# alexrich021/3dvnet

Hardware: AMD Instinct MI355X
Metric: depth maps/sec (256x320, 96 planes, 7 src) (higher is better)
Workload: dtype f32 storage/accumulate; MFMA operands split-bf16x3 (hi*hi+hi*lo+lo*hi, 16 mantissa bits); warp/variance f32 VALU; 1 GPU; cfg2: ScanNet-shape 256x320, 1 ref + 7 src (8 edges/ref), 96 planes, 56x56 plane grid, 32-ch quarter features 64x80; fused warp+variance -> CostRegNet -> soft-argmin depth (rows A1-A6); n_img_per_gpu=71, edges_per_ref=8, parallelism=single GPU, launch=eager, ranks_seen=1

## Files before the change

### 3dvnet_amd/_lib.py

```python
import ctypes
import os

import torch

_HERE = os.path.dirname(os.path.abspath(__file__))
LIB_PATH = os.path.join(_HERE, 'lib3dvnet_hip.so')
ABI_VERSION = 9
PRECISION = {'split_bf16': 0, 'fp32': 1}
LAYOUT = {'reference': 0, 'split': 1, 'cl8': 2}


def precision_code(name):
    try:
        return PRECISION[name]
    except KeyError:
        raise ValueError("precision must be 'split_bf16' or 'fp32', got %r" % (name,))


c_void_p, c_int, c_float, c_double, c_size_t = (ctypes.c_void_p, ctypes.c_int, ctypes.c_float,
                                                ctypes.c_double, ctypes.c_size_t)
c_float_p = ctypes.POINTER(ctypes.c_float)
c_float_pp = ctypes.POINTER(c_float_p)

SIGNATURES = {
    'v3d_version': (c_int, []),
    'v3d_last_error': (ctypes.c_char_p, []),
    'v3d_set_option': (c_int, [ctypes.c_char_p, c_int]),
    'v3d_get_option': (c_int, [ctypes.c_char_p, ctypes.POINTER(c_int)]),
    'v3d_timing_enable': (c_int, [c_int]),
    'v3d_timing_collect': (c_int, [c_int, ctypes.c_char_p, c_int, ctypes.POINTER(c_float),
                                   ctypes.POINTER(c_int)]),
    'v3d_psv_workspace_bytes': (c_size_t, [c_int] * 4),
    'v3d_psv_walk_chunks': (c_int, [c_int] * 4),
    'v3d_psv_variance_f32': (c_int, [c_void_p] * 7 + [c_int] * 8 + [c_double] * 2 + [c_int] * 3 +
                             [c_void_p, c_void_p, c_size_t, c_void_p]),
    'v3d_psv_sample_positions_f32': (c_int, [c_void_p] * 6 + [c_int] * 7 + [c_double] * 2 + [c_int] * 3 +
                                     [c_void_p, c_void_p, c_void_p, c_size_t, c_void_p]),
    'v3d_psv_variance_split': (c_int, [c_void_p] * 7 + [c_int] * 8 + [c_double] * 2 + [c_int] * 3 +
                               [c_void_p, c_void_p, c_size_t, c_void_p]),
    'v3d_psv_variance_cl8': (c_int, [c_void_p] * 7 + [c_int] * 8 + [c_double] * 2 + [c_int] * 3 +
                             [c_void_p, c_void_p, c_size_t, c_void_p]),
    'v3d_costreg_depth_cl8': (c_int, [c_void_p] * 3 + [c_int] * 4 + [c_void_p, c_void_p, c_void_p,
                                                                    c_size_t, c_void_p]),
    'v3d_costreg_pack': (c_int, [c_float_pp] * 5 + [c_float_p, c_float_p, c_int, c_int, c_float,
                                                     ctypes.POINTER(c_void_p)]),
    'v3d_costreg_free': (None, [c_void_p]),
    'v3d_costreg_workspace_bytes': (c_size_t, [c_void_p] + [c_int] * 4),
    'v3d_costreg_depth_f32': (c_int, [c_void_p] * 3 + [c_int] * 4 + [c_void_p, c_void_p, c_int, c_void_p,
                                                                    c_size_t, c_void_p]),
    'v3d_costreg_depth_split': (c_int, [c_void_p] * 3 + [c_int] * 4 + [c_void_p, c_void_p, c_void_p,
                                                                      c_size_t, c_void_p]),
    'v3d_costreg_layer_f32': (c_int, [c_void_p, c_int, c_void_p, c_void_p] + [c_int] * 4 +
                              [c_void_p, c_int, c_void_p]),
    'v3d_costreg_layer_split_workspace_bytes': (c_size_t, [c_int] * 5),
    'v3d_costreg_layer_split_f32': (c_int, [c_void_p, c_int, c_void_p, c_void_p] + [c_int] * 4 +
                                    [c_void_p, c_void_p, c_size_t, c_void_p]),
    'v3d_propagation_pack': (c_int, [c_float_pp] * 5 + [c_int, c_int, c_float, ctypes.POINTER(c_void_p)]),
    'v3d_propagation_free': (None, [c_void_p]),
    'v3d_propagation_up_f32': (c_int, [c_void_p, c_void_p, c_void_p] + [c_int] * 6 + [c_void_p, c_void_p, c_void_p, c_int, c_void_p]),
    'v3d_backproject_workspace_bytes': (c_size_t, [c_int] * 4),
    'v3d_backproject_variance_f32': (c_int, [c_void_p] * 8 + [c_int] * 10 + [c_double, c_int] +
                                     [c_void_p, c_void_p, c_void_p, c_size_t, c_void_p]),
    'v3d_gemm_pack': (c_int, [c_float_p, ctypes.c_longlong, ctypes.c_longlong, ctypes.c_longlong,
                              c_int, c_int, c_int, c_float_p, c_float_p, c_float_p, c_float_p,
                              ctypes.POINTER(c_void_p)]),
    'v3d_gemm_free': (None, [c_void_p]),
    'v3d_gemm_gather_f32': (c_int, [c_void_p, c_int, ctypes.POINTER(c_void_p), ctypes.POINTER(c_void_p),
                                    ctypes.POINTER(c_int), c_int, c_int, c_int, c_float, c_void_p, c_int,
                                    c_int, c_void_p, c_void_p, c_int, c_void_p, c_int, c_int, c_void_p]),
    'v3d_sparse_conv_f32': (c_int, [c_void_p, c_int, c_void_p, c_int, c_void_p, ctypes.c_longlong, c_int, c_float, c_void_p,
                                    c_int, c_int, c_void_p, c_int, c_int, c_void_p]),
    'v3d_fill_f32': (c_int, [c_void_p, c_size_t, c_float, c_void_p]),
    'v3d_pointnet_input_f32': (c_int, [c_void_p] * 5 + [c_int, c_int, c_void_p, c_void_p]),
    'v3d_hash_bytes': (c_size_t, [c_int]),
    'v3d_hash_build': (c_int, [c_void_p, c_int, c_void_p, c_size_t, c_void_p]),
    'v3d_hash_status': (c_int, [c_void_p, c_int, c_void_p]),
    'v3d_sparse_neighbors': (c_int, [c_void_p, c_int, c_void_p, c_int, c_int, c_void_p, c_void_p]),
    'v3d_sparse_interp_workspace_bytes': (c_size_t, [c_int, c_int]),
    'v3d_sparse_interp_f32': (c_int, [c_void_p, c_int, c_void_p, c_int, c_int, c_void_p, c_void_p, c_int,
                                      c_int, c_void_p, c_float, c_void_p, c_int, c_int, c_void_p, c_size_t,
                                      c_void_p]),
    'v3d_edges_csr_workspace_bytes': (c_size_t, [c_int, c_int]),
    'v3d_edges_csr': (c_int, [c_void_p, c_int, c_int, c_int, c_void_p, c_void_p, c_void_p, c_void_p, c_size_t, c_void_p]),
    'v3d_edges_csr_status': (c_int, [c_void_p, c_size_t, c_void_p]),
    'v3d_segment_csr_workspace_bytes': (c_size_t, [c_int]),
    'v3d_segment_csr': (c_int, [c_void_p, c_int, c_int, c_void_p, c_void_p, c_void_p, c_size_t, c_void_p]),
    'v3d_segment_max_f32': (c_int, [c_void_p, c_int, c_void_p, c_void_p, c_int, c_int, c_void_p, c_int, c_void_p]),
    'v3d_sort_unique_workspace_bytes': (c_size_t, [c_int]),
    'v3d_sort_unique_u64': (c_int, [c_void_p, c_int, c_void_p, ctypes.POINTER(c_int), c_void_p, c_size_t, c_void_p]),
    'v3d_strided_keys': (c_int, [c_void_p, c_int, c_int, c_void_p, c_void_p]),
    'v3d_unpack_coords': (c_int, [c_void_p, c_int, c_void_p, c_void_p]),
    'v3d_voxelize_workspace_bytes': (c_size_t, []),
    'v3d_voxel_keys': (c_int, [c_void_p, c_void_p, c_int, c_float, c_void_p, c_void_p, c_size_t, c_void_p]),
    'v3d_voxelize_status': (c_int, [c_void_p, c_size_t, c_void_p]),
    'v3d_lower_bound_u64': (c_int, [c_void_p, c_int, c_void_p, c_int, c_void_p, c_void_p]),
    'v3d_voxel_decode': (c_int, [c_void_p, c_int, c_float, c_float, c_void_p, c_void_p, c_void_p, c_void_p,
                                 c_size_t, c_void_p]),
    'v3d_decoder_fused_f32': (c_int, [ctypes.POINTER(c_void_p), c_void_p, c_void_p, ctypes.POINTER(c_void_p),
                                      ctypes.POINTER(c_int), ctypes.POINTER(c_void_p), ctypes.POINTER(c_int),
                                      ctypes.POINTER(c_int), ctypes.POINTER(c_void_p), ctypes.POINTER(c_float), c_void_p,
                                      c_void_p, c_void_p, c_int, c_int, c_int, c_void_p, c_void_p, c_void_p, c_void_p, c_void_p,
                                      c_size_t, c_void_p]),
    'v3d_decoder_fused_workspace_bytes': (c_size_t, [c_int, c_int]),
    'v3d_conv_pack': (c_int, [c_float_p, c_float_p, c_int, c_int, ctypes.POINTER(c_void_p)]),
    'v3d_conv_free': (None, [c_void_p]),
    'v3d_conv_nhwc_f32': (c_int, [c_void_p, c_void_p] + [c_int] * 7 + [c_void_p, c_void_p, c_void_p]),
    'v3d_depthwise_nhwc_f32': (c_int, [c_void_p] * 3 + [c_int] * 7 + [c_void_p, c_void_p]),
    'v3d_stem_f32': (c_int, [c_void_p] * 3 + [c_int] * 3 + [c_void_p, c_void_p]),
    'v3d_nhwc_to_nchw_f32': (c_int, [c_void_p, c_void_p, c_int, c_int, c_int, c_void_p]),
    'v3d_irb_pack': (c_int, [c_float_p] * 6 + [c_int] * 6 + [ctypes.POINTER(c_void_p)]),
    'v3d_irb_free': (None, [c_void_p]),
    'v3d_irb_supported': (c_int, [c_void_p, c_int, c_int]),
    'v3d_irb_workspace_bytes': (c_size_t, [c_void_p, c_int, c_int, c_int]),
    'v3d_stem_block_pack': (c_int, [c_float_p] * 6 + [ctypes.POINTER(c_void_p)]),
    'v3d_stem_block_f32': (c_int, [c_void_p, c_void_p, c_int, c_int, c_int, c_void_p, c_void_p]),
    'v3d_irb_nhwc_f32': (c_int, [c_void_p, c_void_p, c_int, c_int, c_int, c_void_p, c_void_p, c_size_t, c_void_p]),
    'v3d_fpn_pack': (c_int, [c_float_p] * 4 + [c_int, ctypes.POINTER(c_void_p)]),
    'v3d_fpn_free': (None, [c_void_p]),
    'v3d_fpn_level_f32': (c_int, [c_void_p, c_void_p, c_void_p, c_int, c_int, c_int, c_void_p, c_void_p, c_void_p]),
    'v3d_decoder_head_f32': (c_int, [c_void_p, c_int, c_int, c_int, c_void_p, c_void_p, c_void_p, c_void_p,
                                     c_void_p, c_void_p]),
    'v3d_fusion_workspace_bytes': (c_size_t, [c_int] * 3),
    'v3d_fuse_depths_f32': (c_int, [c_void_p, c_void_p, c_int, c_int, c_int, ctypes.POINTER(c_int), c_int, ctypes.POINTER(c_int),
                                    ctypes.POINTER(c_int), c_double, c_void_p, c_void_p, c_void_p, c_size_t, c_void_p]),
    'v3d_fusion_compact': (c_int, [c_void_p, c_void_p, c_void_p] + [c_int] * 5 + [c_void_p] * 7 + [c_size_t, c_void_p]),
    'v3d_cloud_downsample_workspace_bytes': (c_size_t, [c_int]),
    'v3d_cloud_downsample_f32': (c_int, [c_void_p, c_void_p, c_int, c_int, c_void_p, c_double, c_void_p, c_void_p, c_void_p,
                                         c_void_p, c_size_t, c_void_p]),
    'v3d_cloud_status': (c_int, [c_void_p, c_size_t, ctypes.POINTER(c_int), c_void_p]),
    'v3d_nn_workspace_bytes': (c_size_t, [c_int, c_int]),
    'v3d_nn_query_f32': (c_int, [c_void_p, c_int, c_void_p, c_int, c_void_p, c_void_p, c_void_p, c_size_t, c_void_p]),
    'v3d_cloud_metrics_workspace_bytes': (c_size_t, []),
    'v3d_cloud_metrics_f64': (c_int, [c_void_p, c_int, c_void_p, c_int, c_double, c_void_p, c_void_p, c_size_t, c_void_p]),
    'v3d_tsdf_integrate_f32': (c_int, [c_void_p, c_void_p, c_void_p, c_int, c_int, c_int, c_double, c_float_p, c_double, c_void_p,
                                       c_void_p, c_void_p, c_int, c_int, c_int, c_void_p]),
    'v3d_tsdf_normalize_f32': (c_int, [c_void_p, c_void_p, c_void_p, c_int, c_void_p, c_void_p, c_void_p]),
    'v3d_mesh_workspace_bytes': (c_size_t, [c_int, c_int, c_int]),
    'v3d_mesh_count_f32': (c_int, [c_void_p, c_int, c_int, c_int, c_int, c_void_p, c_void_p, c_size_t, c_void_p]),
    'v3d_mesh_extract_f32': (c_int, [c_void_p, c_void_p, c_int, c_int, c_int, c_double, c_float_p, c_int, c_void_p, c_void_p, c_int,
                                     c_void_p, c_int, c_void_p, c_size_t, c_void_p]),
    'v3d_mesh_render_depth_f32': (c_int, [c_void_p, c_int, c_void_p, c_int, c_void_p, c_int, c_int, c_int, c_double, c_double,
                                          c_double, c_void_p, c_void_p, c_void_p]),
    'v3d_tsdf_resample_f32': (c_int, [c_void_p, c_void_p, c_int, c_int, c_int, c_int, c_double, c_float_p, c_float_p, c_int, c_int,
                                      c_int, c_int, c_float_p, c_void_p, c_void_p, c_void_p]),
    'v3d_volume_resample_nearest': (c_int, [c_void_p, c_int, c_int, c_int, c_int, c_int, c_double, c_float_p, c_float_p, c_int, c_int,
                                            c_int, c_int, c_float_p, c_int, c_void_p, c_void_p, c_void_p]),
    'v3d_costreg_depth_prob': (c_int, [c_void_p, c_void_p, c_int, c_int, c_void_p, c_double, c_double] + [c_int] * 4 +
                               [c_void_p, c_void_p, c_void_p, c_void_p, c_size_t, c_void_p]),
    'v3d_soft_argmin_f32': (c_int, [c_void_p, c_void_p, c_double, c_double] + [c_int] * 4 + [c_void_p, c_void_p, c_void_p]),
    'v3d_confidence_logits_f32': (c_int, [c_void_p, c_void_p, c_double, c_double] + [c_int] * 4 + [c_void_p, c_void_p]),
    'v3d_probability_map_f32': (c_int, [c_void_p, c_void_p, c_double, c_double] + [c_int] * 4 + [c_void_p, c_void_p]),
    'v3d_depth_metrics_workspace_bytes': (c_size_t, [c_int] * 3),
    'v3d_depth_metrics_2d': (c_int, [c_void_p, c_int, c_int, c_void_p, c_void_p, c_void_p, c_int, c_void_p, c_int] + [c_int] * 3 +
                             [c_void_p, c_void_p, c_void_p, c_void_p, c_size_t, c_void_p]),
    'v3d_depth_supervision_workspace_bytes': (c_size_t, [c_int] * 3),
    'v3d_depth_supervision_f32': (c_int, [c_void_p, c_int, c_int, c_int, c_void_p, c_int, c_int, c_void_p, c_void_p, c_float] +
                                  [c_void_p, c_void_p, c_void_p, c_void_p, c_size_t, c_void_p]),
    'v3d_order_stats_workspace_bytes': (c_size_t, [c_int]),
    'v3d_backproject_order_stats_f32': (c_int, [c_void_p, c_void_p, c_int, c_int, c_int, ctypes.POINTER(c_double), c_int, c_void_p,
                                                c_void_p, c_void_p, c_size_t, c_void_p]),
    'v3d_cloud_order_stats_f32': (c_int, [c_void_p, c_int, ctypes.POINTER(c_double), c_int, c_void_p, c_void_p, c_void_p, c_size_t,
                                          c_void_p]),
}


class V3DLibraryError(RuntimeError):
    """lib3dvnet_hip.so is missing / unloadable, or a call returned an error code."""


_ERR_NAMES = {-1: 'V3D_ERR_BAD_SHAPE', -2: 'V3D_ERR_BAD_ARG', -3: 'V3D_ERR_WORKSPACE_TOO_SMALL',
              -4: 'V3D_ERR_HIP', -5: 'V3D_ERR_UNSUPPORTED'}
_lib = None


def load():
    global _lib
    if _lib is not None:
        return _lib
    if not os.path.exists(LIB_PATH):
        raise V3DLibraryError('%s not found: the HIP extension is not built (run '
                              '`python 3dvnet_amd/build.py`); there is no CPU fallback' % LIB_PATH)
    try:
        lib = ctypes.CDLL(LIB_PATH)
    except OSError as e:
        raise V3DLibraryError('cannot load %s: %s' % (LIB_PATH, e))
    for name, (res, args) in SIGNATURES.items():
        try:
            fn = getattr(lib, name)
        except AttributeError:
            raise V3DLibraryError('%s does not export %s' % (LIB_PATH, name))
        fn.restype = res
        fn.argtypes = args
    if lib.v3d_version() != ABI_VERSION:
        raise V3DLibraryError('ABI version mismatch: library %d, binding %d'
# ... 53 lines not shown
```

### 3dvnet_amd/csrc/costreg.hip

```cpp
#include <cstdlib>
#include <type_traits>
#include <vector>

#include "v3d_common.h"
#include "weight_pack.h"

#ifndef V3D_ABLATE
#define V3D_ABLATE 0
#endif

namespace {

typedef float f32x4 __attribute__((ext_vector_type(4)));
typedef float f32x2 __attribute__((ext_vector_type(2)));

enum { kConvS1 = 0, kConvS2 = 1, kDeconvS2 = 2, kConvS1Pair = 3 };

#ifdef V3D_PHASE_TIMING
constexpr int kPhaseSlots = 1 << 16;
__device__ unsigned long long g_phase[8 * kPhaseSlots];
#define PHASE_DECL                                  \
  long long ph_t = __builtin_readcyclecounter();    \
  long long ph_acc[8] = {0, 0, 0, 0, 0, 0, 0, 0}
#define PHASE_MARK(i)                                   \
// ... 1396 lines not shown
    for (int j = 0; j < 4; ++j) acc[i][j] = (f32x4){0.f, 0.f, 0.f, 0.f};
#pragma unroll
  for (int cbi = 0; cbi < NCBI; ++cbi) {
    const int cb = wave + 8 * cbi;
    if (cb < C9::NCB && V3D_C9_ABLATE != 3) {
      const int cz = cb / C9::CY, cy = cb % C9::CY;
#pragma unroll
      for (int dz = 0; dz < 2; ++dz)
#pragma unroll
        for (int dy = 0; dy < 2; ++dy) {
          if constexpr (F32) {
            float bv[8];
#pragma unroll
            for (int sl = 0; sl < 8; ++sl)
              bv[sl] = xf[(4 * (sl & 3) + kq) * C9::FS + ((cz + dz) * C9::VY + (cy + dy)) * C9::VX + jn + (sl >> 2)];
#pragma unroll
            for (int pz = 0; pz < 2; ++pz)
#pragma unroll
              for (int py = 0; py < 2; ++py) {
                if ((pz == 0 || dz == 1) && (py == 0 || dy == 1)) {
                  const int blk = (pz == 1 ? 2 : dz) * 3 + (py == 1 ? 2 : dy);
                  const f32x4 a0 = *reinterpret_cast<const f32x4*>(wff + ((blk * 2 + 0) * 64 + lane) * 4);
                  const f32x4 a1 = *reinterpret_cast<const f32x4*>(wff + ((blk * 2 + 1) * 64 + lane) * 4);
                  f32x4& c = acc[cbi][pz * 2 + py];
#pragma unroll
                  for (int sl = 0; sl < 8; ++sl)
                    c = __builtin_amdgcn_mfma_f32_16x16x4f32(sl < 4 ? a0[sl] : a1[sl - 4], bv[sl], c, 0, 0, 0);
                }
              }
            continue;
          }
          const int slot = (((cz + dz) * C9::VY + (cy + dy)) * C9::VX + jn + (kq >> 1)) * 2 + (kq & 1);
          const bf16x8 b_hi = __builtin_bit_cast(bf16x8, xh[slot]);
          const bf16x8 b_lo = __builtin_bit_cast(bf16x8, xl[slot]);
#pragma unroll
          for (int pz = 0; pz < 2; ++pz)
#pragma unroll
            for (int py = 0; py < 2; ++py) {
              if ((pz == 0 || dz == 1) && (py == 0 || dy == 1)) {
                const int blk = (pz == 1 ? 2 : dz) * 3 + (py == 1 ? 2 : dy);
                const bf16x8 a_hi = __builtin_bit_cast(bf16x8, wfr[(blk * 2) * 64 + lane]);
                const bf16x8 a_lo = __builtin_bit_cast(bf16x8, wfr[(blk * 2 + 1) * 64 + lane]);
                f32x4& c = acc[cbi][pz * 2 + py];
                c = __builtin_amdgcn_mfma_f32_16x16x32_bf16(a_hi, b_hi, c, 0, 0, 0);
                c = __builtin_amdgcn_mfma_f32_16x16x32_bf16(a_hi, b_lo, c, 0, 0, 0);
                c = __builtin_amdgcn_mfma_f32_16x16x32_bf16(a_lo, b_hi, c, 0, 0, 0);
              }
            }
        }
    }
  }
  PHASE_MARK(2);
  __syncthreads();
  PHASE_MARK(3);

  {
    float bias[4];
#pragma unroll
    for (int r = 0; r < 4; ++r) bias[r] = p.bias9[cbase + r];
#pragma unroll
    for (int cbi = 0; cbi < NCBI; ++cbi) {
      const int cb = wave + 8 * cbi;
      if (cb < C9::NCB && jn < C9::CX) {
        const int cz = cb / C9::CY, cy = cb % C9::CY;
#pragma unroll
        for (int rb = 0; rb < 4; ++rb) {
          const int hz = 2 * cz + (rb >> 1), hy = 2 * cy + (rb & 1), hx = 2 * jn + px;
          const int gz = oz0 - 1 + hz, gy = oy0 - 1 + hy, gx = ox0 - 1 + hx;
          const bool inside = gz >= 0 && gz < p.D && gy >= 0 && gy < p.H && gx >= 0 && gx < p.W;
          float skv[4];
          if constexpr (F32) {
#pragma unroll
            for (int r = 0; r < 4; ++r) skv[r] = skf[cbi][rb][r];
          } else {
            const u32x2 sh = skh[cbi][rb], sl = skl[cbi][rb];
            skv[0] = __uint_as_float(sh.x << 16) + __uint_as_float(sl.x << 16);
            skv[1] = __uint_as_float(sh.x & 0xffff0000u) + __uint_as_float(sl.x & 0xffff0000u);
            skv[2] = __uint_as_float(sh.y << 16) + __uint_as_float(sl.y << 16);
            skv[3] = __uint_as_float(sh.y & 0xffff0000u) + __uint_as_float(sl.y & 0xffff0000u);
          }
          float val[4];
#pragma unroll
          for (int r = 0; r < 4; ++r) val[r] = inside ? fmaxf(acc[cbi][rb][r] + bias[r], 0.f) + skv[r] : 0.f;
#pragma unroll
          for (int rp = 0; rp < 2; ++rp)
            *reinterpret_cast<f32x2*>(u9s + ((((cbase >> 1) + rp) * (C9::HD * C9::HH) + hz * C9::HH + hy) * C9::RS + hx) * 2) =
                (f32x2){val[2 * rp], val[2 * rp + 1]};
        }
      }
    }
  }
  PHASE_MARK(4);
  __syncthreads();
  PHASE_MARK(5);

  {
    const int z = wave >> 1, y = (wave & 1) * 4 + (lane >> 4), xp = lane & 15;
    if (xp < C9::TW / 2) {
      f32x2 o0[3] = {{0.f, 0.f}, {0.f, 0.f}, {0.f, 0.f}}, o1[3] = {{0.f, 0.f}, {0.f, 0.f}, {0.f, 0.f}};
      const f32x2* wp2 = reinterpret_cast<const f32x2*>(p.wprob);
#pragma unroll 1
      for (int cp = 0; cp < (V3D_C9_ABLATE == 1 ? 0 : V3D_C9_ABLATE == 2 ? 1 : 4); ++cp) {
#pragma unroll
        for (int ky = 0; ky < 3; ++ky) {
#pragma unroll
          for (int kz = 0; kz < 3; ++kz) {
            const f32x2* row = reinterpret_cast<const f32x2*>(u9s) +
                               (cp * (C9::HD * C9::HH) + (z + kz) * C9::HH + (y + ky)) * C9::RS + 2 * xp;
            const f32x4 q0 = *reinterpret_cast<const f32x4*>(row), q1 = *reinterpret_cast<const f32x4*>(row + 2);
            const f32x2 a0 = {q0.x, q0.y}, a1 = {q0.z, q0.w}, a2 = {q1.x, q1.y}, a3 = {q1.z, q1.w};
            const f32x2* wk = wp2 + (cp * 27 + (kz * 3 + ky) * 3);
            const f32x2 w0 = wk[0], w1 = wk[1], w2 = wk[2];
            o0[kz] += a0 * w0; o1[kz] += a1 * w0;
            o0[kz] += a1 * w1; o1[kz] += a2 * w1;
            o0[kz] += a2 * w2; o1[kz] += a3 * w2;
          }
        }
      }
      const f32x2 s0 = (o0[0] + o0[1]) + o0[2], s1 = (o1[0] + o1[1]) + o1[2];
      const int gz = oz0 + z, gy = oy0 + y, gx = ox0 + 2 * xp;
      if (gz < p.D && gy < p.H && gx < p.W) {
        const float bsv = p.bprob[0];
        const f32x2 res = {s0.x + s0.y + bsv, s1.x + s1.y + bsv};
        float* o = p.out + ((size_t)n * out_plane + (size_t)(gz * p.H) * p.W) + (unsigned)(__umul24(gy, p.W) + gx);
        if (gx + 1 < p.W && (p.W & 1) == 0) {
          *reinterpret_cast<f32x2*>(o) = res;
        } else {
          o[0] = res.x;
          if (gx + 1 < p.W) o[1] = res.y;
        }
      }
    }
  }
  PHASE_MARK(6);
  PHASE_FLUSH;
}

__global__ __launch_bounds__(256) void encode_split_kernel(const float* __restrict__ in, u32x4* __restrict__ out, int C,
                                                           size_t plane, size_t total) {
  const size_t i = (size_t)blockIdx.x * 256 + threadIdx.x;
  if (i >= total) return;
  const size_t sp = i % plane, ng = i / plane;
  const float* src = in + (ng * 8) * plane + sp;
  float v[8];
#pragma unroll
  for (int c = 0; c < 8; ++c) v[c] = src[(size_t)c * plane];
  u32x2 ha, la, hb, lb;
  split4(v[0], v[1], v[2], v[3], ha, la);
  split4(v[4], v[5], v[6], v[7], hb, lb);
  out[(ng * 2) * plane + sp] = (u32x4){ha.x, ha.y, hb.x, hb.y};
  out[(ng * 2 + 1) * plane + sp] = (u32x4){la.x, la.y, lb.x, lb.y};
}

__global__ __launch_bounds__(256) void soft_argmin_kernel(const float* __restrict__ reg,
                                                          const float* __restrict__ vals,
                                                          float* __restrict__ depth, int n, int D,
                                                          int HW) {
  const size_t gid = (size_t)blockIdx.x * 256 + threadIdx.x;
  if (gid >= (size_t)n * HW) return;
  const int b = gid / HW, pix = gid % HW;
  const float* col = reg + (size_t)b * D * HW + pix;
  float m = -INFINITY, num = 0.f, den = 0.f;
  auto step = [&](float xin, float val) __attribute__((always_inline)) {
    const float x = -xin;
    if (x > m) {
      const float sc = expf(m - x);
      num *= sc; den *= sc; m = x;
    }
    const float ex = expf(x - m);
    num += val * ex;
    den += ex;
  };
  int d = 0;
  for (; d + 8 <= D; d += 8) {
    float x[8];
#pragma unroll
    for (int i = 0; i < 8; ++i) x[i] = __builtin_nontemporal_load(col + (size_t)(d + i) * HW);
#pragma unroll
    for (int i = 0; i < 8; ++i) step(x[i], vals[d + i]);
  }
  for (; d < D; ++d) step(col[(size_t)d * HW], vals[d]);
  const float e = num / den;
  depth[gid] = e;
}

#ifndef V3D_L0_CFG
#define V3D_L0_CFG kConvS1Pair, 32, 8, 4, 8, 28, 4, 3
#endif
typedef ConvCfg<V3D_L0_CFG> L0;
typedef ConvCfg<kConvS1Pair, 16, 8, 4, 8, 28, 4, 3> L0_16;
#ifndef V3D_L1_CFG
#define V3D_L1_CFG kConvS2, 8, 16, 2, 4, 28, 4
#endif
typedef ConvCfg<V3D_L1_CFG> L1;
#ifndef V3D_L2_CFG
#define V3D_L2_CFG kConvS1, 16, 16, 4, 4, 28, 8
#endif
typedef ConvCfg<V3D_L2_CFG> L2;
typedef ConvCfg<kConvS2, 16, 32, 2, 7, 14, 4> L3;
typedef ConvCfg<kConvS1, 32, 32, 4, 7, 14, 8> L4;
typedef ConvCfg<kConvS2, 32, 64, 2, 4, 7, 8> L5;
typedef ConvCfg<kConvS1, 64, 64, 2, 4, 7, 16> L6;
typedef ConvCfg<kDeconvS2, 64, 32, 4, 8, 14, 16> L7;
#ifndef V3D_L8_CFG
#define V3D_L8_CFG kDeconvS2, 32, 16, 4, 8, 28, 8
#endif
typedef ConvCfg<V3D_L8_CFG> L8;
#ifndef V3D_L9_CFG
#define V3D_L9_CFG kDeconvS2, 16, 8, 4, 8, 28, 16, 3
#endif
typedef ConvCfg<V3D_L9_CFG> L9;

struct LayerDesc { int mode, cin, cout, ck; };
const LayerDesc kLayers[10] = {
    {L0::MODE, 32, 8, L0::CK},   {L1::MODE, 8, 16, L1::CK},   {L2::MODE, 16, 16, L2::CK},
    {kConvS2, 16, 32, L3::CK},  {kConvS1, 32, 32, L4::CK},  {kConvS2, 32, 64, L5::CK},
    {kConvS1, 64, 64, L6::CK},  {kDeconvS2, 64, 32, L7::CK}, {kDeconvS2, 32, 16, L8::CK},
    {kDeconvS2, 16, 8, L9::CK}};

template <class C>
int launch_conv(const char* name, const float* in, const float* wp, const float* bias,
                const float* skip, float* out, int n, int Di, int Hi, int Wi, hipStream_t s) {
  ConvParams p;
  p.in = in; p.wp = wp; p.bias = bias; p.skip = skip; p.out = out; p.n = n;
  p.Di = Di; p.Hi = Hi; p.Wi = Wi;
  if (C::S1LIKE) { p.Do = Di; p.Ho = Hi; p.Wo = Wi; }
  else if (C::MODE == kConvS2) { p.Do = (Di - 1) / 2 + 1; p.Ho = (Hi - 1) / 2 + 1; p.Wo = (Wi - 1) / 2 + 1; }
  else { p.Do = 2 * Di; p.Ho = 2 * Hi; p.Wo = 2 * Wi; }
  p.ntz = (p.Do + C::TD - 1) / C::TD; p.nty = (p.Ho + C::TH - 1) / C::TH; p.ntx = (p.Wo + C::TW - 1) / C::TW;
  p.relu = 1;
  p.zy_order = 0;
  const long long blocks = (long long)n * p.ntz * p.nty * p.ntx;
  V3D_REQUIRE(blocks > 0 && blocks < (1ll << 31), V3D_ERR_BAD_SHAPE, "conv3d: bad grid");
  V3D_REQUIRE((long long)C::CK * Di * Hi * Wi < (1ll << 31), V3D_ERR_BAD_SHAPE,
              "conv3d: input volume too large for 32-bit tile offsets");
  {
    v3d::TimedScope ts(name, s);
    constexpr bool kVecOk = C::MODE == kConvS1Pair && C::PF && C::TW % 4 == 0 && C::IW <= 61;
    const bool vec = kVecOk && Wi % 4 == 0 && (reinterpret_cast<size_t>(in) & 15) == 0;
    if constexpr (kVecOk) {
      if (vec) conv3d_mfma_kernel<C, true><<<(unsigned)blocks, 256, 0, s>>>(p);
      else conv3d_mfma_kernel<C, false><<<(unsigned)blocks, 256, 0, s>>>(p);
    } else {
      conv3d_mfma_kernel<C, false><<<(unsigned)blocks, 256, 0, s>>>(p);
    }
  }
  V3D_CHECK_LAUNCH("conv3d_mfma_kernel");
  return V3D_OK;
}

}

namespace {
#ifndef V3D_C0_WAVES
#define V3D_C0_WAVES 8
#endif
constexpr int kC0Waves = V3D_C0_WAVES;
int launch_conv0_bf16(bool split_in, bool split_out, const float* in, const float* wbf, const float* bias, const float* skip, float* out, int n,
                      int Di, int Hi, int Wi, hipStream_t s) {
  ConvParams p;
  p.in = in; p.wp = wbf; p.bias = bias; p.skip = skip; p.out = out; p.n = n;
  p.Di = Di; p.Hi = Hi; p.Wi = Wi; p.Do = Di; p.Ho = Hi; p.Wo = Wi;
  p.ntz = (Di + C0::TD - 1) / C0::TD; p.nty = (Hi + C0::TH - 1) / C0::TH; p.ntx = (Wi + C0::TW - 1) / C0::TW;
  p.relu = 1;
  p.zy_order = tile_order(p.ntx, p.nty);
  const long long blocks = (long long)n * p.ntz * p.nty * p.ntx;
  V3D_REQUIRE(blocks > 0 && blocks < (1ll << 31), V3D_ERR_BAD_SHAPE, "conv0: bad grid");
  V3D_REQUIRE((long long)8 * Di * Hi * Wi < (1ll << 31), V3D_ERR_BAD_SHAPE, "conv0: input volume too large");
  static bool lds_opted[4][64] = {};
  const void* const kernels[4] = {(const void*)conv0_bf16x2_kernel<false, false, 4>, (const void*)conv0_bf16x2_kernel<true, false, 4>,
                                  (const void*)conv0_bf16x2_kernel<true, true, kC0Waves>, (const void*)conv0_bf16x2_kernel<false, true, 4>};
  for (int k = 0; k < 4; ++k)
    if (const int rc = v3d::opt_in_dynamic_lds(kernels[k], (int)C0::LDS_BYTES, lds_opted[k]); rc != V3D_OK) return rc;
  {
    v3d::TimedScope ts("costreg_conv0", s);
#ifdef V3D_C0_PERSIST
    const unsigned grid = v3d::persistent_grid(blocks, 2);
#else
    const unsigned grid = (unsigned)((blocks + 7) / 8 * 8);
#endif
    if (split_in && split_out) conv0_bf16x2_kernel<true, true, kC0Waves><<<grid, 64 * kC0Waves, C0::LDS_BYTES, s>>>(p);
    else if (split_in) conv0_bf16x2_kernel<true, false, 4><<<grid, 256, C0::LDS_BYTES, s>>>(p);
    else if (split_out) conv0_bf16x2_kernel<false, true, 4><<<grid, 256, C0::LDS_BYTES, s>>>(p);
    else conv0_bf16x2_kernel<false, false, 4><<<grid, 256, C0::LDS_BYTES, s>>>(p);
  }
  V3D_CHECK_LAUNCH("conv0_bf16x2_kernel");
  return V3D_OK;
}
}

namespace {
template <class C>
int launch_convg(const char* name, const void* in, const float* wbf, const float* bias, float* out_f32, void* out_split,
                 int n, int Di, int Hi, int Wi, hipStream_t s) {
  ConvGParams p;
  p.in = in; p.wp = wbf; p.bias = bias; p.out_f32 = out_f32; p.out_split = out_split; p.n = n;
  p.Di = Di; p.Hi = Hi; p.Wi = Wi;
  p.Do = (Di - 1) / C::S + 1; p.Ho = (Hi - 1) / C::S + 1; p.Wo = (Wi - 1) / C::S + 1;
  p.ntz = (p.Do + C::TD - 1) / C::TD; p.nty = (p.Ho + C::TH - 1) / C::TH; p.ntx = (p.Wo + C::TW - 1) / C::TW;
  const long long blocks = (long long)n * p.ntz * p.nty * p.ntx;
  V3D_REQUIRE(blocks > 0 && blocks < (1ll << 31), V3D_ERR_BAD_SHAPE, "%s: bad grid", name);
  V3D_REQUIRE(((C::OUT & kOutF32) == 0 || out_f32) && ((C::OUT & kOutSplit) == 0 || out_split), V3D_ERR_BAD_ARG,
              "%s: missing output buffer", name);
  p.m_tx = v3d::magic_u32((unsigned long long)blocks, (unsigned)p.ntx);
  p.m_ty = v3d::magic_u32((unsigned long long)blocks / p.ntx + 1, (unsigned)p.nty);
  p.m_tz = v3d::magic_u32((unsigned long long)blocks / p.ntx / p.nty + 1, (unsigned)p.ntz);
  V3D_REQUIRE(Di < (1 << 12) && Hi < (1 << 12) && Wi < (1 << 12) && (long long)Di * Hi * Wi < (1ll << 24), V3D_ERR_BAD_SHAPE,
              "%s: volume %d x %d x %d too large for 32-bit slot offsets", name, Di, Hi, Wi);
  static bool lds_opted[64] = {};
  if (const int rc = v3d::opt_in_dynamic_lds((const void*)convg_bf16x2_kernel<C>, (int)C::LDS_BYTES, lds_opted); rc != V3D_OK) return rc;
  {
    v3d::TimedScope ts(name, s);
    unsigned grid = (unsigned)((blocks * C::NCG + 7) / 8 * 8);
    if (C::PERSIST) {
      static int wgs_per_cu = 0;
      if (wgs_per_cu == 0) {
        int nb = 0;
        V3D_CHECK_HIP(hipOccupancyMaxActiveBlocksPerMultiprocessor(&nb, (const void*)convg_bf16x2_kernel<C>, 256, C::LDS_BYTES));
        wgs_per_cu = nb > 0 ? nb : 1;
      }
      grid = v3d::persistent_grid(blocks * C::NCG, wgs_per_cu);
    }
    convg_bf16x2_kernel<C><<<grid, 256, C::LDS_BYTES, s>>>(p, p.bias);
  }
  V3D_CHECK_LAUNCH(name);
  return V3D_OK;
}
}

namespace {
template <class C>
int launch_deconvg(const char* name, const void* in, const float* wbf, const float* bias, const float* skip, float* out_f32,
                   void* out_split, int n, int Di, int Hi, int Wi, hipStream_t s) {
  DeconvGParams p;
// ... 134 lines not shown

void pack_prob(const float* prob_w, float* out) {
  for (int cp = 0; cp < 4; ++cp)
    for (int t = 0; t < 27; ++t)
      for (int e = 0; e < 2; ++e) out[((size_t)cp * 27 + t) * 2 + e] = prob_w[(cp * 2 + e) * 27 + t];
}
}

extern "C" int v3d_costreg_pack(const float* const* conv_w, const float* const* bn_w,
                                const float* const* bn_b, const float* const* bn_m,
                                const float* const* bn_v, const float* prob_w, const float* prob_b,
                                int in_channels, int base, float eps,
                                v3d_costreg_weights** out_handle) {
  V3D_REQUIRE(conv_w && bn_w && bn_b && bn_m && bn_v && prob_w && prob_b && out_handle,
              V3D_ERR_BAD_ARG, "v3d_costreg_pack: null argument");
  V3D_REQUIRE((in_channels == 32 || in_channels == 16) && base == 8, V3D_ERR_UNSUPPORTED,
              "v3d_costreg_pack: CostRegNet(32, 8) and CostRegNet(16, 8) are built (got %d, %d)", in_channels, base);
  v3d_costreg_weights* h = new v3d_costreg_weights();
  h->in_channels = in_channels; h->base = base;
  v3d::HostImage img;
  std::vector<float> wf[10];
  for (int l = 0; l < 10; ++l) {
    LayerDesc L = kLayers[l];
    if (l == 0) L.cin = in_channels;
    const v3d::BnFold bn(bn_w[l], bn_b[l], bn_m[l], bn_v[l], eps, L.cout);
    wf[l] = L.mode == kDeconvS2 ? bn.weights(conv_w[l], L.cin, 27) : bn.weights(conv_w[l], 1, (size_t)L.cin * 27);
    h->wp_ofs[l] = img.reserve(tile_image_floats(L));
    h->bias_ofs[l] = img.reserve(L.cout);
    pack_tile_image(L, wf[l].data(), img.at(h->wp_ofs[l]));
    memcpy(img.at(h->bias_ofs[l]), bn.bias.data(), L.cout * sizeof(float));
  }
  h->c0bf_ofs = img.reserve((size_t)C0::NCH * C0::WU32);
  pack_conv0_split(wf[0].data(), in_channels, img.words(h->c0bf_ofs));
  h->c0f32_ofs = img.reserve((size_t)4 * 9 * 8 * 64);
  pack_conv0_f32(wf[0].data(), in_channels, img.at(h->c0f32_ofs));
  h->c9bf_ofs = img.reserve((size_t)C9::WU32);
  h->c9f32_ofs = img.reserve((size_t)C9::WF32);
  pack_conv9(wf[9].data(), img.words(h->c9bf_ofs), img.at(h->c9f32_ofs));
  for (int l = 1; l <= 8; ++l) {
    const int cin = kLayers[l].cin, cout = kLayers[l].cout;
    size_t& ofs = l <= 6 ? h->cgbf_ofs[l] : h->dgbf_ofs[l - 7];
    ofs = img.reserve((size_t)(cout / 16) * (cin / 8) * (l <= 6 ? 9 : 12) * 2 * kLoWords);
    if (l <= 6) pack_convg(wf[l].data(), cin, cout, img.words(ofs));
    else pack_deconvg(wf[l].data(), cin, cout, img.words(ofs));
  }
  h->prob_w2_ofs = img.reserve((size_t)base * 27);
  pack_prob(prob_w, img.at(h->prob_w2_ofs));
  h->prob_b_ofs = img.reserve(1);
  *img.at(h->prob_b_ofs) = prob_b[0];
  h->total = img.data.size();
  return v3d::finish_pack(h, img.data.data(), h->total * sizeof(float), "weights", out_handle);
}

extern "C" void v3d_costreg_free(v3d_costreg_weights* h) { v3d::release(h); }

static int run_layer(const v3d_costreg_weights* h, int layer, const float* in, const float* skip,
                     float* out, int n, int Di, int Hi, int Wi, int precision, hipStream_t s) {
  const float* wp = h->dev + h->wp_ofs[layer];
  const float* bias = h->dev + h->bias_ofs[layer];
  switch (layer) {
    case 0: {
      if (h->in_channels == 16) {
        V3D_REQUIRE(precision == V3D_PRECISION_FP32, V3D_ERR_UNSUPPORTED,
                    "costreg: the per-layer conv0 of CostRegNet(16, 8) is built for V3D_PRECISION_FP32 only (the chain entry points "
                    "cover both precisions)");
        return launch_conv<L0_16>("costreg_conv0", in, wp, bias, skip, out, n, Di, Hi, Wi, s);
      }
      if (precision == V3D_PRECISION_FP32) return launch_conv<L0>("costreg_conv0", in, wp, bias, skip, out, n, Di, Hi, Wi, s);
      return launch_conv0_bf16(false, false, in, h->dev + h->c0bf_ofs, bias, skip, out, n, Di, Hi, Wi, s);
    }
    case 1: return launch_conv<L1>("costreg_conv1", in, wp, bias, skip, out, n, Di, Hi, Wi, s);
    case 2: return launch_conv<L2>("costreg_conv2", in, wp, bias, skip, out, n, Di, Hi, Wi, s);
    case 3: return launch_conv<L3>("costreg_conv3", in, wp, bias, skip, out, n, Di, Hi, Wi, s);
    case 4: return launch_conv<L4>("costreg_conv4", in, wp, bias, skip, out, n, Di, Hi, Wi, s);
    case 5: return launch_conv<L5>("costreg_conv5", in, wp, bias, skip, out, n, Di, Hi, Wi, s);
    case 6: return launch_conv<L6>("costreg_conv6", in, wp, bias, skip, out, n, Di, Hi, Wi, s);
    case 7: return launch_conv<L7>("costreg_conv7", in, wp, bias, skip, out, n, Di, Hi, Wi, s);
    case 8: return launch_conv<L8>("costreg_conv8", in, wp, bias, skip, out, n, Di, Hi, Wi, s);
    case 9: return launch_conv<L9>("costreg_conv9", in, wp, bias, skip, out, n, Di, Hi, Wi, s);
  }
  return v3d::fail(V3D_ERR_BAD_ARG, "costreg: layer %d out of range", layer);
}

extern "C" int v3d_costreg_layer_f32(const v3d_costreg_weights* h, int layer, const float* in,
                                     const float* skip, int n, int Di, int Hi, int Wi, float* out,
                                     int precision, void* stream) {
  V3D_REQUIRE(h && in && out, V3D_ERR_BAD_ARG, "v3d_costreg_layer_f32: null argument");
  V3D_REQUIRE(n > 0 && Di > 0 && Hi > 0 && Wi > 0, V3D_ERR_BAD_SHAPE, "v3d_costreg_layer_f32: bad shape");
  V3D_REQUIRE(precision == V3D_PRECISION_SPLIT_BF16 || precision == V3D_PRECISION_FP32, V3D_ERR_BAD_ARG,
              "v3d_costreg_layer_f32: unknown precision %d", precision);
  return run_layer(h, layer, in, skip, out, n, Di, Hi, Wi, precision, (hipStream_t)stream);
}

extern "C" size_t v3d_costreg_layer_split_workspace_bytes(int n, int cin, int Di, int Hi, int Wi) {
  if (n <= 0 || cin <= 0 || Di <= 0 || Hi <= 0 || Wi <= 0) return 0;
  return v3d::align_up((size_t)n * cin * Di * Hi * Wi * sizeof(float), 256);
}

extern "C" int v3d_costreg_layer_split_f32(const v3d_costreg_weights* h, int layer, const float* in, const float* skip,
                                           int n, int Di, int Hi, int Wi, float* out, void* workspace,
                                           size_t workspace_bytes, void* stream) {
  static const int cins[9] = {32, 8, 16, 16, 32, 32, 64, 64, 32};
  V3D_REQUIRE(h && in && out && workspace, V3D_ERR_BAD_ARG, "v3d_costreg_layer_split_f32: null argument");
  V3D_REQUIRE(layer >= 1 && layer <= 8, V3D_ERR_BAD_ARG, "v3d_costreg_layer_split_f32: layer %d (1..8: conv1..conv8)", layer);
  V3D_REQUIRE(n > 0 && Di > 0 && Hi > 0 && Wi > 0, V3D_ERR_BAD_SHAPE, "v3d_costreg_layer_split_f32: bad shape");
  V3D_REQUIRE(layer < 7 || skip, V3D_ERR_BAD_ARG, "v3d_costreg_layer_split_f32: conv7 / conv8 need the skip tensor");
  const int cin = cins[layer];
  V3D_REQUIRE(workspace_bytes >= v3d_costreg_layer_split_workspace_bytes(n, cin, Di, Hi, Wi), V3D_ERR_WORKSPACE_TOO_SMALL,
              "v3d_costreg_layer_split_f32: workspace too small");
  hipStream_t s = (hipStream_t)stream;
  const size_t plane = (size_t)Di * Hi * Wi, total = (size_t)n * (cin / 8) * plane;
  encode_split_kernel<<<(unsigned)((total + 255) / 256), 256, 0, s>>>(in, (u32x4*)workspace, cin, plane, total);
  V3D_CHECK_LAUNCH("encode_split_kernel");
  const float* w = h->dev + (layer <= 6 ? h->cgbf_ofs[layer] : h->dgbf_ofs[layer - 7]);
  const float* bias = h->dev + h->bias_ofs[layer];
  switch (layer) {
    case 1: return launch_convg<CG<8, 16, 2, 14, kOutF32>>("costreg_conv1", workspace, w, bias, out, nullptr, n, Di, Hi, Wi, s);
    case 2: return launch_convg<CG<16, 16, 1, 14, kOutF32>>("costreg_conv2", workspace, w, bias, out, nullptr, n, Di, Hi, Wi, s);
    case 3: return launch_convg<CG<16, 32, 2, 14, kOutF32>>("costreg_conv3", workspace, w, bias, out, nullptr, n, Di, Hi, Wi, s);
    case 4: return launch_convg<CG<32, 32, 1, 14, kOutF32>>("costreg_conv4", workspace, w, bias, out, nullptr, n, Di, Hi, Wi, s);
    case 5: return launch_convg<CG<32, 64, 2, 8, kOutF32>>("costreg_conv5", workspace, w, bias, out, nullptr, n, Di, Hi, Wi, s);
    case 6: return launch_convg<CG<64, 64, 1, 8, kOutF32>>("costreg_conv6", workspace, w, bias, out, nullptr, n, Di, Hi, Wi, s);
    case 7: return launch_deconvg<DG<64, 32, 8, kOutF32>>("costreg_conv7", workspace, w, bias, skip, out, nullptr, n, Di, Hi, Wi, s);
    default: return launch_deconvg<DG<32, 16, 14, kOutF32>>("costreg_conv8", workspace, w, bias, skip, out, nullptr, n, Di, Hi, Wi, s);
  }
}

namespace {
struct WsPlan { size_t c0, c1, c2, c3, c4, c5, c6, u7, u8, u9, reg, enc, total; };
WsPlan plan_ws(int n, int D, int h, int w) {
  const size_t V0 = (size_t)D * h * w, V1 = V0 / 8, V2 = V1 / 8, V3 = V2 / 8;
  WsPlan p; size_t o = 0;
  auto take = [&](size_t nf) { size_t r = o; o += v3d::align_up(nf * sizeof(float), 256); return r; };
  p.c0 = take(n * 8 * V0); p.c1 = take(n * 16 * V1); p.c2 = take(n * 16 * V1);
  p.c3 = take(n * 32 * V2); p.c4 = take(n * 32 * V2); p.c5 = take(n * 64 * V3);
  p.c6 = take(n * 64 * V3); p.u7 = take(n * 32 * V2); p.u8 = take(n * 16 * V1);
  p.u9 = take(n * 8 * V0); p.reg = take(n * V0);
  p.enc = take(32 * V0);
  p.total = o;
  return p;
}
}

extern "C" size_t v3d_costreg_workspace_bytes(const v3d_costreg_weights*, int n_ref, int D, int h, int w) {
  if (n_ref <= 0 || D <= 0 || h <= 0 || w <= 0) return 0;
  return plan_ws(n_ref, D, h, w).total;
}

namespace {
int launch_soft_argmin(const float* xreg, const float* depth_vals, float* depth, int n, int D, int H, int W, hipStream_t s) {
  const size_t npix = (size_t)n * H * W;
  {
    v3d::TimedScope ts("soft_argmin", s);
    soft_argmin_kernel<<<(unsigned)((npix + 255) / 256), 256, 0, s>>>(xreg, depth_vals, depth, n, D, H * W);
  }
  V3D_CHECK_LAUNCH("soft_argmin_kernel");
  return V3D_OK;
}

struct ProbOut {
  float* prob = nullptr;
  double depth_start = 0., depth_interval = 0.;
};

int launch_depth_tail(const float* xreg, const float* depth_vals, float* depth, const ProbOut& po, int n, int D, int H, int W,
                      hipStream_t s) {
  if (!po.prob) return launch_soft_argmin(xreg, depth_vals, depth, n, D, H, W, s);
  return v3d::launch_soft_argmin_prob(xreg, depth_vals, depth, po.prob, po.depth_start, po.depth_interval, n, D, H, W, s);
}

int launch_conv9_prob(bool f32, const v3d_costreg_weights* h, const float* u8, const float* c0, float* xreg, int n, int D, int H, int W,
                      hipStream_t s) {
  C9Params q;
  q.u8 = u8; q.c0 = c0; q.wbf = h->dev + (f32 ? h->c9f32_ofs : h->c9bf_ofs); q.bias9 = h->dev + h->bias_ofs[9];
  q.wprob = h->dev + h->prob_w2_ofs; q.bprob = h->dev + h->prob_b_ofs; q.out = xreg;
  q.n = n; q.D = D; q.H = H; q.W = W;
  q.ntz = (D + C9::TD - 1) / C9::TD; q.nty = (H + C9::TH - 1) / C9::TH; q.ntx = (W + C9::TW - 1) / C9::TW;
  q.zy_order = tile_order(q.ntx, q.nty);
  const long long blocks = (long long)n * q.ntz * q.nty * q.ntx;
  V3D_REQUIRE(blocks < (1ll << 31), V3D_ERR_BAD_SHAPE, "conv9+prob: grid too large");
  V3D_REQUIRE((long long)D * H * W < (1ll << 26) && D < (1 << 12) && H < (1 << 12) && W < (1 << 12), V3D_ERR_BAD_SHAPE,
              "conv9+prob: volume %d x %d x %d too large for 32-bit offsets", D, H, W);
  q.m_tx = v3d::magic_u32((unsigned long long)blocks, (unsigned)q.ntx);
  q.m_t1 = v3d::magic_u32((unsigned long long)blocks / q.ntx + 1, (unsigned)(q.zy_order ? q.ntz : q.nty));
  q.m_t2 = v3d::magic_u32((unsigned long long)blocks / q.ntx / (q.zy_order ? q.ntz : q.nty) + 1, (unsigned)(q.zy_order ? q.nty : q.ntz));
  {
    v3d::TimedScope ts(f32 ? "costreg_conv9_prob_f32" : "costreg_conv9_prob", s);
    if (f32) conv9_prob_kernel<true><<<(unsigned)blocks, 512, 0, s>>>(q);
    else conv9_prob_kernel<false><<<(unsigned)blocks, 512, 0, s>>>(q);
  }
  V3D_CHECK_LAUNCH("conv9_prob_kernel");
  return V3D_OK;
}

int run_split_tail(const v3d_costreg_weights* h, const WsPlan& ws, char* base, const float* depth_vals, int n, int D, int H, int W,
                   float* depth, float* xreg, const ProbOut& po, hipStream_t s) {
  const size_t V1 = (size_t)D * H * W / 8;
  auto F = [&](size_t o) { return (float*)(base + o); };
  float* const c2s = F(ws.u9);
  float* const c4s = c2s + (size_t)n * 16 * V1;
  auto W_ = [&](int l) { return h->dev + h->cgbf_ofs[l]; };
  auto B_ = [&](int l) { return h->dev + h->bias_ofs[l]; };
#ifdef V3D_PHASE_TIMING
  const int stop_after = v3d::option(v3d::kOptStopAfter);
#else
  const int stop_after = 99;
#endif
  int rc = V3D_OK;
  if (stop_after < 1) return rc;
  if (v3d::option(v3d::kOptC12March) != 0) {
    rc = v3d::launch_conv12z(F(ws.c0), W_(1), W_(2), B_(1), B_(2), c2s, n, D, H, W, s);
  } else if ((rc = launch_convg<CG<8, 16, 2, 14, kOutSplit>>("costreg_conv1", F(ws.c0), W_(1), B_(1), nullptr, F(ws.c1), n, D, H, W,
                                                              s)) == V3D_OK) {
    rc = launch_convg<CG<16, 16, 1, 14, kOutSplit>>("costreg_conv2", F(ws.c1), W_(2), B_(2), nullptr, c2s, n, D / 2, H / 2, W / 2, s);
  }
  if (rc != V3D_OK || stop_after < 3) return rc;
  if ((rc = launch_convg<CG<16, 32, 2, 14, kOutSplit>>("costreg_conv3", c2s, W_(3), B_(3), nullptr, F(ws.c3), n, D / 2, H / 2, W / 2,
                                                       s)) != V3D_OK || stop_after < 4) return rc;
  if ((rc = launch_convg<CG<32, 32, 1, 14, kOutSplit>>("costreg_conv4", F(ws.c3), W_(4), B_(4), nullptr, c4s, n, D / 4, H / 4, W / 4,
                                                       s)) != V3D_OK || stop_after < 5) return rc;
  if ((rc = launch_convg<CG<32, 64, 2, 8, kOutSplit>>("costreg_conv5", c4s, W_(5), B_(5), nullptr, F(ws.c5), n, D / 4, H / 4, W / 4,
                                                      s)) != V3D_OK || stop_after < 6) return rc;
  if ((rc = launch_convg<CG<64, 64, 1, 8, kOutSplit>>("costreg_conv6", F(ws.c5), W_(6), B_(6), nullptr, F(ws.c6), n, D / 8, H / 8,
                                                      W / 8, s)) != V3D_OK || stop_after < 7) return rc;
  if ((rc = launch_deconvg<DG<64, 32, 8, kOutSplit, true>>("costreg_conv7", F(ws.c6), h->dev + h->dgbf_ofs[0], B_(7), c4s, nullptr,
                                                           F(ws.u7), n, D / 8, H / 8, W / 8, s)) != V3D_OK || stop_after < 8) return rc;
  if ((rc = launch_deconvg<DG<32, 16, 14, kOutSplit, true>>("costreg_conv8", F(ws.u7), h->dev + h->dgbf_ofs[1], B_(8), c2s, nullptr,
                                                            F(ws.u8), n, D / 4, H / 4, W / 4, s)) != V3D_OK || stop_after < 9) return rc;
  if ((rc = launch_conv9_prob(false, h, F(ws.u8), F(ws.c0), xreg, n, D, H, W, s)) != V3D_OK || stop_after < 10) return rc;
  return launch_depth_tail(xreg, depth_vals, depth, po, n, D, H, W, s);
}
}

static int costreg_depth_impl(int in_layout, const v3d_costreg_weights* h, const float* var,
                              const float* depth_vals, int n, int D, int H, int W,
                              float* depth, float* reg, int precision, void* workspace,
                              size_t workspace_bytes, void* stream, const ProbOut& po = ProbOut()) {
  V3D_REQUIRE(precision == V3D_PRECISION_SPLIT_BF16 || precision == V3D_PRECISION_FP32, V3D_ERR_BAD_ARG,
              "v3d_costreg_depth_f32: unknown precision %d", precision);
  V3D_REQUIRE(h && var && depth_vals && depth && workspace, V3D_ERR_BAD_ARG,
              "v3d_costreg_depth_f32: null argument");
  V3D_REQUIRE(n > 0 && D > 0 && H > 0 && W > 0 && D % 8 == 0 && H % 8 == 0 && W % 8 == 0,
              V3D_ERR_BAD_SHAPE, "v3d_costreg_depth_f32: D,h,w must be positive multiples of 8 (got %d,%d,%d)", D, H, W);
  const WsPlan ws = plan_ws(n, D, H, W);
  V3D_REQUIRE(workspace_bytes >= ws.total, V3D_ERR_WORKSPACE_TOO_SMALL,
              "v3d_costreg_depth_f32: workspace %zu < %zu", workspace_bytes, ws.total);
  hipStream_t s = (hipStream_t)stream;
  char* base = (char*)workspace;
  auto F = [&](size_t o) { return (float*)(base + o); };
  float* xreg = reg ? reg : F(ws.reg);
  int rc;
#define RUN(layer, in, skip, out, d, hh, ww) \
  if ((rc = run_layer(h, layer, in, skip, out, n, d, hh, ww, V3D_PRECISION_FP32, s)) != V3D_OK) return rc;
  const bool generic = precision == V3D_PRECISION_FP32;
  const bool split_in = in_layout == 1, cl8_in = in_layout == 2;
  V3D_REQUIRE(!generic || !split_in, V3D_ERR_UNSUPPORTED, "V3D_PRECISION_FP32 needs an fp32 variance volume");
  V3D_REQUIRE(h->in_channels == 32 || in_layout == 0, V3D_ERR_UNSUPPORTED,
              "CostRegNet(16, 8) takes the variance volume in the reference layout (the hand-off formats are defined for 32 channels)");
  V3D_REQUIRE(generic || !cl8_in, V3D_ERR_UNSUPPORTED, "the fp32 channel-last volume is the input of V3D_PRECISION_FP32");
  if (generic) {
    if (cl8_in) {
      if ((rc = v3d::launch_conv0z(true, var, h->dev + h->c0f32_ofs, h->dev + h->bias_ofs[0], F(ws.c0), n, D, H, W, s)) != V3D_OK)
        return rc;
    } else {
      RUN(0, var, nullptr, F(ws.c0), D, H, W);
    }
    RUN(1, F(ws.c0), nullptr, F(ws.c1), D, H, W);
    RUN(2, F(ws.c1), nullptr, F(ws.c2), D / 2, H / 2, W / 2);
  } else {
    if (split_in) {
      if ((rc = v3d::launch_conv0z(false, var, h->dev + h->c0bf_ofs, h->dev + h->bias_ofs[0], F(ws.c0), n, D, H, W, s)) != V3D_OK) return rc;
    } else {
      const int cin = h->in_channels, ngrp = cin / 8;
      const size_t V0 = (size_t)D * H * W, total = (size_t)ngrp * V0;
      if (ngrp < 4) V3D_CHECK_HIP(hipMemsetAsync((char*)F(ws.enc) + (size_t)ngrp * 2 * V0 * 16, 0, (size_t)(4 - ngrp) * 2 * V0 * 16, s));
      for (int i = 0; i < n; ++i) {
        encode_split_kernel<<<(unsigned)((total + 255) / 256), 256, 0, s>>>(var + (size_t)i * cin * V0, (u32x4*)F(ws.enc), cin, V0, total);
        V3D_CHECK_LAUNCH("encode_split_kernel");
        if ((rc = v3d::launch_conv0z(false, F(ws.enc), h->dev + h->c0bf_ofs, h->dev + h->bias_ofs[0], F(ws.c0) + (size_t)i * 8 * V0, 1, D, H,
                                     W, s)) != V3D_OK) return rc;
      }
    }
    return run_split_tail(h, ws, base, depth_vals, n, D, H, W, depth, xreg, po, s);
  }
  RUN(3, F(ws.c2), nullptr, F(ws.c3), D / 2, H / 2, W / 2);
  RUN(4, F(ws.c3), nullptr, F(ws.c4), D / 4, H / 4, W / 4);
  RUN(5, F(ws.c4), nullptr, F(ws.c5), D / 4, H / 4, W / 4);
  RUN(6, F(ws.c5), nullptr, F(ws.c6), D / 8, H / 8, W / 8);
  RUN(7, F(ws.c6), F(ws.c4), F(ws.u7), D / 8, H / 8, W / 8);
  RUN(8, F(ws.u7), F(ws.c2), F(ws.u8), D / 4, H / 4, W / 4);
  if ((rc = launch_conv9_prob(true, h, F(ws.u8), F(ws.c0), xreg, n, D, H, W, s)) != V3D_OK) return rc;
#undef RUN
  return launch_depth_tail(xreg, depth_vals, depth, po, n, D, H, W, s);
}

extern "C" int v3d_costreg_depth_f32(const v3d_costreg_weights* h, const float* var, const float* depth_vals, int n,
                                     int D, int H, int W, float* depth, float* reg, int precision, void* workspace,
                                     size_t workspace_bytes, void* stream) {
  return costreg_depth_impl(0, h, var, depth_vals, n, D, H, W, depth, reg, precision, workspace, workspace_bytes,
                            stream);
}

extern "C" int v3d_costreg_depth_cl8(const v3d_costreg_weights* h, const void* var_cl8, const float* depth_vals,
                                     int n, int D, int H, int W, float* depth, float* reg, void* workspace,
                                     size_t workspace_bytes, void* stream) {
  return costreg_depth_impl(2, h, (const float*)var_cl8, depth_vals, n, D, H, W, depth, reg, V3D_PRECISION_FP32, workspace,
                            workspace_bytes, stream);
}

extern "C" int v3d_costreg_depth_split(const v3d_costreg_weights* h, const void* var_split, const float* depth_vals,
                                       int n, int D, int H, int W, float* depth, float* reg, void* workspace,
                                       size_t workspace_bytes, void* stream) {
  return costreg_depth_impl(1, h, (const float*)var_split, depth_vals, n, D, H, W, depth, reg,
                            V3D_PRECISION_SPLIT_BF16, workspace, workspace_bytes, stream);
}

extern "C" int v3d_costreg_depth_prob(const v3d_costreg_weights* h, const void* var, int in_layout, int precision,
                                      const float* depth_vals, double depth_start, double depth_interval, int n, int D, int H,
                                      int W, float* depth, float* reg, float* prob, void* workspace, size_t workspace_bytes,
                                      void* stream) {
  V3D_REQUIRE(in_layout == V3D_LAYOUT_REFERENCE || in_layout == V3D_LAYOUT_SPLIT || in_layout == V3D_LAYOUT_CL8, V3D_ERR_BAD_ARG,
              "v3d_costreg_depth_prob: unknown input layout %d", in_layout);
  const float ds = (float)depth_start, di = (float)depth_interval;
  V3D_REQUIRE(std::isfinite(ds) && std::isfinite(di) && di != 0.f, V3D_ERR_BAD_ARG,
              "v3d_costreg_depth_prob: depth_start = %g / depth_interval = %g must be finite fp32 numbers, the interval not zero",
              depth_start, depth_interval);
  V3D_REQUIRE(D < (1 << 24), V3D_ERR_BAD_SHAPE, "v3d_costreg_depth_prob: D = %d too large", D);
  ProbOut po;
  po.prob = prob; po.depth_start = depth_start; po.depth_interval = depth_interval;
  return costreg_depth_impl(in_layout, h, (const float*)var, depth_vals, n, D, H, W, depth, reg, precision, workspace,
                            workspace_bytes, stream, po);
}

extern "C" int v3d_soft_argmin_f32(const float* x_reg, const float* depth_vals, double depth_start, double depth_interval, int n,
                                   int D, int H, int W, float* depth, float* prob, void* stream) {
  V3D_REQUIRE(x_reg && depth_vals && depth, V3D_ERR_BAD_ARG, "v3d_soft_argmin_f32: null argument");
  V3D_REQUIRE(n > 0 && D > 0 && H > 0 && W > 0 && D < (1 << 24) && (long long)H * W < (1ll << 31) &&
                  ((long long)n * H * W + 255) / 256 < (1ll << 31),
              V3D_ERR_BAD_SHAPE, "v3d_soft_argmin_f32: n, D, h, w = %d, %d, %d, %d", n, D, H, W);
  const float ds = (float)depth_start, di = (float)depth_interval;
  V3D_REQUIRE(!prob || (std::isfinite(ds) && std::isfinite(di) && di != 0.f), V3D_ERR_BAD_ARG,
              "v3d_soft_argmin_f32: depth_start = %g / depth_interval = %g must be finite fp32 numbers, the interval not zero",
              depth_start, depth_interval);
  ProbOut po;
  po.prob = prob; po.depth_start = depth_start; po.depth_interval = depth_interval;
  return launch_depth_tail(x_reg, depth_vals, depth, po, n, D, H, W, (hipStream_t)stream);
}

#ifdef V3D_PHASE_TIMING
extern "C" int v3d_debug_phase_read(unsigned long long* out8_host, int n_blocks) {
  V3D_CHECK_HIP(hipDeviceSynchronize());
  std::vector<unsigned long long> h((size_t)8 * kPhaseSlots);
  V3D_CHECK_HIP(hipMemcpyFromSymbol(h.data(), HIP_SYMBOL(g_phase), h.size() * sizeof(unsigned long long)));
  for (int i = 0; i < 8; ++i) out8_host[i] = 0;
  for (int b = 0; b < n_blocks && b < kPhaseSlots; ++b)
    for (int i = 0; i < 8; ++i) out8_host[i] += h[(size_t)b * 8 + i];
  return V3D_OK;
}
#endif
```

### 3dvnet_amd/csrc/edges.hip

```cpp
#include "v3d_common.h"

namespace {

constexpr int kThreads = 1024, kWaves = kThreads / 64;

struct CsrMeta {
  int magic;
  int error;
  int n_ref;
  int pad;
};
constexpr int kMagic = 0x43535231;
constexpr int kLdsImgs = 4096, kLdsEdges = 8192;

__device__ __forceinline__ int block_inclusive_sum(int v, int* s_wave, int& total) {
  const int lane = threadIdx.x & 63, wave = threadIdx.x >> 6;
#pragma unroll
  for (int o = 1; o < 64; o <<= 1) {
    const int u = __shfl_up(v, o, 64);
    if (lane >= o) v += u;
  }
  __syncthreads();
  if (lane == 63) s_wave[wave] = v;
  __syncthreads();
  int base = 0, tot = 0;
#pragma unroll
  for (int w = 0; w < kWaves; ++w) {
    const int x = s_wave[w];
    if (w < wave) base += x;
    tot += x;
  }
  total = tot;
  return v + base;
}

__global__ __launch_bounds__(kThreads) void edges_csr_kernel(const long long* __restrict__ edges, int n_edges, int n_img,
                                                              int n_ref_expected, int* __restrict__ ref_img,
                                                              int* __restrict__ edge_ofs, int* __restrict__ edge_src,
                                                              CsrMeta* __restrict__ meta, int* rank,
                                                              int* __restrict__ count) {
  __shared__ int s_wave[kWaves];
  __shared__ int s_err;
  __shared__ int s_rank[kLdsImgs];
  __shared__ int s_er[kLdsEdges];
  const bool small = n_img <= kLdsImgs && n_edges <= kLdsEdges;
  if (small) rank = s_rank;
  const int tid = threadIdx.x, lane = tid & 63, wave = tid >> 6;
  const long long* const e_ref = edges;
  const long long* const e_src = edges + n_edges;
  if (tid == 0) s_err = 0;
  for (int i = tid; i < n_img; i += kThreads) rank[i] = 0;
  __syncthreads();
  int bad = 0;
  for (int e = tid; e < n_edges; e += kThreads) {
    const long long r = e_ref[e], s = e_src[e];
    if (r < 0 || r >= n_img || s < 0 || s >= n_img) bad = 1;
    else rank[r] = 1;
  }
  if (bad) s_err = 2;
  __syncthreads();
  const int per = (n_img + kThreads - 1) / kThreads;
  const int lo = min(tid * per, n_img), hi = min(lo + per, n_img);
  int sum = 0;
  for (int i = lo; i < hi; ++i) sum += rank[i];
  int n_ref;
  int run = block_inclusive_sum(sum, s_wave, n_ref) - sum;
  for (int i = lo; i < hi; ++i) {
    const int f = rank[i];
    rank[i] = f ? run : -1;
    if (f && run < n_ref_expected) ref_img[run] = i;
    run += f;
  }
  int err = s_err | (n_ref != n_ref_expected ? 1 : 0);
  if (tid == 0) { meta->magic = kMagic; meta->error = err; meta->n_ref = n_ref; }
  __syncthreads();
  if (err) {
    for (int r = tid; r <= n_ref_expected; r += kThreads) edge_ofs[r] = 0;
    for (int r = tid; r < n_ref_expected; r += kThreads) ref_img[r] = 0;
    return;
  }
  if (small) {
    for (int e = tid; e < n_edges; e += kThreads) s_er[e] = rank[e_ref[e]];
    __syncthreads();
  }
  auto edge_rank = [&](int e) __attribute__((always_inline)) { return small ? s_er[e] : rank[e_ref[e]]; };
  for (int r = wave; r < n_ref; r += kWaves) {
    int c = 0;
    for (int e0 = 0; e0 < n_edges; e0 += 64) {
      const int e = e0 + lane;
      const bool hit = e < n_edges && edge_rank(e) == r;
      c += __builtin_popcountll(__ballot(hit));
    }
    if (lane == 0) count[r] = c;
  }
  __syncthreads();
  const int per_r = (n_ref + kThreads - 1) / kThreads;
  const int rlo = min(tid * per_r, n_ref), rhi = min(rlo + per_r, n_ref);
  sum = 0;
  for (int r = rlo; r < rhi; ++r) sum += count[r];
  int n_counted;
  run = block_inclusive_sum(sum, s_wave, n_counted) - sum;
  for (int r = rlo; r < rhi; ++r) { edge_ofs[r] = run; run += count[r]; }
  if (tid == 0) edge_ofs[n_ref] = n_counted;
  __syncthreads();
  for (int r = wave; r < n_ref; r += kWaves) {
    int pos = edge_ofs[r];
    for (int e0 = 0; e0 < n_edges; e0 += 64) {
      const int e = e0 + lane;
      const bool hit = e < n_edges && edge_rank(e) == r;
      const unsigned long long m = __ballot(hit);
      if (hit) edge_src[pos + __builtin_popcountll(m & ((1ull << lane) - 1ull))] = (int)e_src[e];
      pos += __builtin_popcountll(m);
    }
  }
}

}

extern "C" size_t v3d_edges_csr_workspace_bytes(int n_img, int n_ref) {
  return sizeof(CsrMeta) + ((size_t)(n_img > 0 ? n_img : 0) + (size_t)(n_ref > 0 ? n_ref : 0)) * sizeof(int);
}

extern "C" int v3d_edges_csr(const int64_t* edges, int n_edges, int n_img, int n_ref, int32_t* ref_img, int32_t* edge_ofs,
                             int32_t* edge_src, void* workspace, size_t workspace_bytes, void* stream) {
  V3D_REQUIRE(edges && ref_img && edge_ofs && edge_src && workspace, V3D_ERR_BAD_ARG, "v3d_edges_csr: null pointer");
  V3D_REQUIRE(n_edges > 0 && n_img > 0 && n_ref > 0 && n_ref <= n_img, V3D_ERR_BAD_SHAPE,
              "v3d_edges_csr: n_edges=%d n_img=%d n_ref=%d", n_edges, n_img, n_ref);
  V3D_REQUIRE(workspace_bytes >= v3d_edges_csr_workspace_bytes(n_img, n_ref), V3D_ERR_WORKSPACE_TOO_SMALL,
              "v3d_edges_csr: workspace %zu < %zu bytes", workspace_bytes, v3d_edges_csr_workspace_bytes(n_img, n_ref));
  hipStream_t s = (hipStream_t)stream;
  CsrMeta* meta = (CsrMeta*)workspace;
  int* rank = (int*)(meta + 1);
  int* count = rank + n_img;
  {
    v3d::TimedScope ts("edges_csr", s);
    edges_csr_kernel<<<1, kThreads, 0, s>>>((const long long*)edges, n_edges, n_img, n_ref, ref_img, edge_ofs, edge_src, meta,
                                            rank, count);
  }
  V3D_CHECK_LAUNCH("edges_csr_kernel");
  return V3D_OK;
}

extern "C" int v3d_edges_csr_status(const void* workspace, size_t workspace_bytes, void* stream) {
  V3D_REQUIRE(workspace && workspace_bytes >= sizeof(CsrMeta), V3D_ERR_BAD_ARG, "v3d_edges_csr_status: not a CSR workspace");
  CsrMeta h;
  V3D_CHECK_HIP(hipMemcpyAsync(&h, workspace, sizeof(h), hipMemcpyDeviceToHost, (hipStream_t)stream));
  V3D_CHECK_HIP(hipStreamSynchronize((hipStream_t)stream));
  V3D_REQUIRE(h.magic == kMagic, V3D_ERR_BAD_ARG, "v3d_edges_csr_status: not a CSR workspace");
  V3D_REQUIRE((h.error & 2) == 0, V3D_ERR_BAD_SHAPE, "v3d_edges_csr: an edge names an image outside [0, n_img)");
  V3D_REQUIRE((h.error & 1) == 0, V3D_ERR_BAD_SHAPE,
              "v3d_edges_csr: the edge list holds %d distinct reference images, not the number the caller passed", h.n_ref);
  return V3D_OK;
}
```

### 3dvnet_amd/csrc/psv_variance.hip

```cpp
#include <cstdlib>

#include <vector>

#include "bf16_split.h"
#include "v3d_common.h"

namespace {

constexpr int kThreads = 256;
constexpr int kPix = 64;
constexpr int kDB = 4;
constexpr int kMaxE = 8;

struct PsvParams {
  const float* featT;
  const float* K;
  const float* R;
  const float* t;
  const int* ref_img;
  const int* edge_ofs;
  const int* edge_src;
  float* var;
  const float* camp;
  int n_img, n_ref, Hf, Wf, H, W, D, h, w, n_ptile;
  double x_step, y_step, z_start, z_step, z_end;
  float rWm1, rHm1;
  unsigned m_dseg, m_ptile, m_w;
  int n_dchunk, walk, n_dseg;
  int skip;
};


template <int C>
__global__ __launch_bounds__(256) void transpose_channel_last_kernel(const float* __restrict__ in,
                                                                      float* __restrict__ out,
                                                                      int HW) {
  __shared__ float tile[C][kPix + 1];
  const int img = blockIdx.y;
  const int p0 = blockIdx.x * kPix;
  const float* src = in + (size_t)img * C * HW;
  float* dst = out + (size_t)img * HW * C;
  for (int i = threadIdx.x; i < C * kPix; i += 256) {
    int c = i / kPix, p = i % kPix;
    tile[c][p] = (p0 + p < HW) ? src[(size_t)c * HW + p0 + p] : 0.f;
  }
  __syncthreads();
  for (int i = threadIdx.x; i < C * kPix; i += 256) {
    int p = i / C, c = i % C;
    if (p0 + p < HW) dst[(size_t)(p0 + p) * C + c] = tile[c][p];
  }
}

__host__ __device__ constexpr int kTailCells(int Wf) { return 2 * (Wf + 2) + 16; }

template <int C>
__global__ __launch_bounds__(256) void transpose_bordered_kernel(const float* __restrict__ in, float* __restrict__ out, int Hf,
                                                                  int Wf, int n_img) {
  __shared__ float tile[C][kPix + 1];
  const int img = blockIdx.y;
  const int Wp = Wf + 2, HW = Hf * Wf, n_cell = (Hf + 2) * Wp;
  const int q0 = blockIdx.x * kPix;
  const float* src = in + (size_t)img * C * HW;
  float* dst = out + (size_t)img * n_cell * C;
  for (int i = threadIdx.x; i < C * kPix; i += 256) {
    const int c = i / kPix, q = q0 + i % kPix;
    const int yb = q / Wp, xb = q - yb * Wp;
    const bool inside = q < n_cell && yb >= 1 && yb <= Hf && xb >= 1 && xb <= Wf;
    tile[c][i % kPix] = inside ? src[(size_t)c * HW + (yb - 1) * Wf + xb - 1] : 0.f;
  }
  __syncthreads();
  for (int i = threadIdx.x; i < C * kPix; i += 256) {
    const int px = i / C, c = i % C;
    if (q0 + px < n_cell) dst[(size_t)(q0 + px) * C + c] = tile[c][px];
  }
  if (img == n_img - 1 && blockIdx.x == 0) {
    float* tail = out + (size_t)n_img * n_cell * C;
    for (int i = threadIdx.x; i < kTailCells(Wf) * C; i += 256) tail[i] = 0.f;
  }
}

#ifdef V3D_PHASE_TIMING
constexpr int kPhaseSlots = 1 << 16;
__device__ unsigned long long g_psv_phase[8 * kPhaseSlots];
#define PHASE_DECL                                  \
  long long ph_t = __builtin_readcyclecounter();    \
  long long ph_acc[8] = {0, 0, 0, 0, 0, 0, 0, 0}
#define PHASE_MARK(i)                                   \
  do {                                                  \
    long long t_ = __builtin_readcyclecounter();        \
    ph_acc[i] += t_ - ph_t;                             \
    ph_t = t_;                                          \
  } while (0)
#define PHASE_FLUSH                                                                                       \
  do {                                                                                                    \
    if (threadIdx.x == 0 && blockIdx.x < kPhaseSlots)                                                     \
      for (int i_ = 0; i_ < 8; ++i_) g_psv_phase[blockIdx.x * 8 + i_] = (unsigned long long)ph_acc[i_];   \
  } while (0)
#else
#define PHASE_DECL
#define PHASE_MARK(i)
#define PHASE_FLUSH
#endif

constexpr int kCamStride = 36;

__global__ void cam_setup_kernel(const float* __restrict__ K, const float* __restrict__ R,
                                 const float* __restrict__ t, float* __restrict__ camp, int n_img) {
  const int img = blockIdx.x * blockDim.x + threadIdx.x;
  if (img >= n_img) return;
  const float* Kp = K + img * 9;
  const float* Rp = R + img * 9;
  const float* tp = t + img * 3;
  float* o = camp + img * kCamStride;
  double a = Kp[0], bb = Kp[1], c = Kp[2], d = Kp[3], e = Kp[4], f = Kp[5], g = Kp[6], hh = Kp[7], i = Kp[8];
  double det = a * (e * i - f * hh) - bb * (d * i - f * g) + c * (d * hh - e * g);
  double id = 1.0 / det;
  o[0] = (float)((e * i - f * hh) * id);
  o[1] = (float)((c * hh - bb * i) * id);
  o[2] = (float)((bb * f - c * e) * id);
  o[3] = (float)((f * g - d * i) * id);
  o[4] = (float)((a * i - c * g) * id);
  o[5] = (float)((c * d - a * f) * id);
  o[6] = (float)((d * hh - e * g) * id);
  o[7] = (float)((bb * g - a * hh) * id);
  o[8] = (float)((a * e - bb * d) * id);
  for (int k = 0; k < 9; ++k) o[9 + k] = Rp[k];
  for (int k = 0; k < 3; ++k) o[18 + k] = tp[k];
  for (int r = 0; r < 3; ++r)
    for (int j = 0; j < 4; ++j) {
      const float b0 = j < 3 ? Rp[0 * 3 + j] : tp[0], b1 = j < 3 ? Rp[1 * 3 + j] : tp[1], b2 = j < 3 ? Rp[2 * 3 + j] : tp[2];
      o[24 + r * 4 + j] = v3d::add_rn(v3d::add_rn(v3d::mul_rn(Kp[r * 3 + 0], b0), v3d::mul_rn(Kp[r * 3 + 1], b1)),
                                    v3d::mul_rn(Kp[r * 3 + 2], b2));
    }
}

struct TapInfo {
  float w00, w01, w10, w11;
  unsigned b00;
  unsigned pad[3];
};

template <unsigned CB>
__device__ __forceinline__ TapInfo make_taps(float ix, float iy, int Wf, int Hf, int first_cell) {
  ix = fminf(fmaxf(ix, -1.f), (float)Wf);
  iy = fminf(fmaxf(iy, -1.f), (float)Hf);
  const float x0 = floorf(ix), y0 = floorf(iy);
  const float x1 = x0 + 1.f, y1 = y0 + 1.f;
  const float wx0 = x1 - ix, wx1 = ix - x0, wy0 = y1 - iy, wy1 = iy - y0;
  TapInfo ti;
  ti.w00 = v3d::mul_rn(wx0, wy0); ti.w01 = v3d::mul_rn(wx1, wy0);
  ti.w10 = v3d::mul_rn(wx0, wy1); ti.w11 = v3d::mul_rn(wx1, wy1);
  ti.b00 = (unsigned)(first_cell + ((int)y0 + 1) * (Wf + 2) + (int)x0 + 1) * CB;
  return ti;
}

typedef float f32x4 __attribute__((ext_vector_type(4)));
typedef unsigned int u32x2 __attribute__((ext_vector_type(2)));
typedef unsigned int u32x4 __attribute__((ext_vector_type(4)));

using v3d::bf16_rne;
using v3d::pack_bf16x2;

template <int C, bool SPLIT>
__global__ __launch_bounds__(64) void psv_variance_kernel(PsvParams p) {
  constexpr int kThreads = 64, kPix = kThreads / 4;
  constexpr int LP = C / 4;
  constexpr int PPP = kThreads / LP;
  constexpr int NPASS = kPix / PPP;
  static_assert(kPix % PPP == 0, "tile");

  __shared__ TapInfo s_tap[kMaxE * kPix];
  __shared__ __attribute__((aligned(16))) float s_out[C][kPix + 1];
  __shared__ float s_ref[24];
  __shared__ float s_P[kMaxE][12];

  const int tid = threadIdx.x;
  const int n_dchunk = (p.D + kDB - 1) / kDB;
  int b = v3d::xcd_contiguous_block();
  const int ptile = b % p.n_ptile; b /= p.n_ptile;
  const int dchunk = b % n_dchunk;
  const int r = b / n_dchunk;
  const int P = p.h * p.w;
  const int e_begin = p.edge_ofs[r], e_end = p.edge_ofs[r + 1];
  const int ne = e_end - e_begin;
  const int ref = p.ref_img[r];

  if (tid < 21) s_ref[tid] = p.camp[ref * kCamStride + tid];

  const int cg = tid % LP;
  const int pix_in_pass = tid / LP;

  const int px1 = tid % kPix;
  const int gp1 = ptile * kPix + px1;
  float xf = 0.f, yf = 0.f;
  {
    int gy = gp1 / p.w, gx = gp1 % p.w;
    xf = (p.w > 1 && gx == p.w - 1) ? (float)(p.W - 1) : (float)((double)gx * p.x_step);
    yf = (p.h > 1 && gy == p.h - 1) ? (float)(p.H - 1) : (float)((double)gy * p.y_step);
  }
  const float Wm1 = (float)(p.W - 1), Hm1 = (float)(p.H - 1);
  const float rWm1 = (float)(1.0 / (double)(p.W - 1)), rHm1 = (float)(1.0 / (double)(p.H - 1));
  const float Wfm1 = (float)(p.Wf - 1), Hfm1 = (float)(p.Hf - 1);

  PHASE_DECL;
  for (int dd = 0; dd < kDB; ++dd) {
    const int d = dchunk * kDB + dd;
    if (d >= p.D) break;
    const float z = (d == p.D - 1 && p.D > 1) ? (float)p.z_end
                                               : (float)(p.z_start + (double)d * p.z_step);
    float acc_s[NPASS][4], acc_q[NPASS][4];
#pragma unroll
    for (int a = 0; a < NPASS; ++a)
#pragma unroll
      for (int k = 0; k < 4; ++k) acc_s[a][k] = acc_q[a][k] = 0.f;

    for (int ec = 0; ec < ne; ec += kMaxE) {
      const int nec = min(kMaxE, ne - ec);
      __syncthreads();
      PHASE_MARK(0);
      if (dd == 0 || ne > kMaxE) {
        for (int i = tid; i < nec * 12; i += kThreads)
          s_P[i / 12][i % 12] = p.camp[p.edge_src[e_begin + ec + i / 12] * kCamStride + 24 + i % 12];
      }
      __syncthreads();
      PHASE_MARK(1);
      {
        float X, Y, Z;
        v3d::world_point(s_ref, xf, yf, z, X, Y, Z);
        for (int e = tid / kPix; e < nec; e += kThreads / kPix) {
          float ix, iy;
          v3d::sample_position(s_P[e], X, Y, Z, Wm1, rWm1, Hm1, rHm1, Wfm1, Hfm1, ix, iy);
          const TapInfo ti = make_taps<4 * C>(ix, iy, p.Wf, p.Hf, p.edge_src[e_begin + ec + e] * (p.Hf + 2) * (p.Wf + 2));
          s_tap[e * kPix + px1] = ti;
        }
      }
      PHASE_MARK(2);
      __syncthreads();
      PHASE_MARK(3);
#pragma unroll
      for (int a = 0; a < NPASS; ++a) {
        const int px = a * PPP + pix_in_pass;
        for (int e = 0; e < nec; ++e) {
          const TapInfo ti = s_tap[e * kPix + px];
          float4 s;
          {
            const char* fb = reinterpret_cast<const char*>(p.featT);
            const unsigned cgb = cg * 16, rowb = (unsigned)(p.Wf + 2) * (4 * C);
            const float4 v00 = *reinterpret_cast<const float4*>(fb + (size_t)(ti.b00 + cgb));
            const float4 v01 = *reinterpret_cast<const float4*>(fb + (size_t)(ti.b00 + cgb) + 4 * C);
            const float4 v10 = *reinterpret_cast<const float4*>(fb + (size_t)(ti.b00 + rowb + cgb));
            const float4 v11 = *reinterpret_cast<const float4*>(fb + (size_t)(ti.b00 + rowb + cgb) + 4 * C);
            s.x = v3d::mul_rn(v00.x, ti.w00); s.y = v3d::mul_rn(v00.y, ti.w00);
            s.z = v3d::mul_rn(v00.z, ti.w00); s.w = v3d::mul_rn(v00.w, ti.w00);
            s.x = __builtin_fmaf(v01.x, ti.w01, s.x); s.y = __builtin_fmaf(v01.y, ti.w01, s.y);
            s.z = __builtin_fmaf(v01.z, ti.w01, s.z); s.w = __builtin_fmaf(v01.w, ti.w01, s.w);
            s.x = __builtin_fmaf(v10.x, ti.w10, s.x); s.y = __builtin_fmaf(v10.y, ti.w10, s.y);
            s.z = __builtin_fmaf(v10.z, ti.w10, s.z); s.w = __builtin_fmaf(v10.w, ti.w10, s.w);
            s.x = __builtin_fmaf(v11.x, ti.w11, s.x); s.y = __builtin_fmaf(v11.y, ti.w11, s.y);
            s.z = __builtin_fmaf(v11.z, ti.w11, s.z); s.w = __builtin_fmaf(v11.w, ti.w11, s.w);
          }
          acc_s[a][0] = v3d::add_rn(acc_s[a][0], s.x); acc_s[a][1] = v3d::add_rn(acc_s[a][1], s.y);
          acc_s[a][2] = v3d::add_rn(acc_s[a][2], s.z); acc_s[a][3] = v3d::add_rn(acc_s[a][3], s.w);
          acc_q[a][0] = __builtin_fmaf(s.x, s.x, acc_q[a][0]); acc_q[a][1] = __builtin_fmaf(s.y, s.y, acc_q[a][1]);
          acc_q[a][2] = __builtin_fmaf(s.z, s.z, acc_q[a][2]); acc_q[a][3] = __builtin_fmaf(s.w, s.w, acc_q[a][3]);
        }
      }
    }
    PHASE_MARK(4);
    const float cnt = (float)max(ne, 1);
    if constexpr (SPLIT) {
      static_assert(!SPLIT || C == 32, "split layout is defined for 32 channels");
      u32x2* const s_sp = reinterpret_cast<u32x2*>(&s_out[0][0]);
      const int chunk = cg >> 1, half = cg & 1;
#pragma unroll
      for (int a = 0; a < NPASS; ++a) {
        const int px = a * PPP + pix_in_pass;
        unsigned h[4], l[4];
#pragma unroll
        for (int k = 0; k < 4; ++k) {
          const float avg = acc_s[a][k] / cnt;
          const float avg_sq = acc_q[a][k] / cnt;
          const float v = v3d::sub_rn(avg_sq, v3d::mul_rn(avg, avg));
          h[k] = bf16_rne(v);
          l[k] = bf16_rne(v - __uint_as_float(h[k] << 16));
        }
        s_sp[(((chunk * 2 + 0) * (kPix + 1)) + px) * 2 + half] = (u32x2){h[0] | (h[1] << 16), h[2] | (h[3] << 16)};
        s_sp[(((chunk * 2 + 1) * (kPix + 1)) + px) * 2 + half] = (u32x2){l[0] | (l[1] << 16), l[2] | (l[3] << 16)};
      }
      __syncthreads();
      u32x4* const out = reinterpret_cast<u32x4*>(p.var);
      const u32x4* const s_q = reinterpret_cast<const u32x4*>(s_sp);
      for (int i = tid; i < 8 * kPix; i += kThreads) {
        const int g = i / kPix, px = i % kPix;
        const int gp = ptile * kPix + px;
        if (gp < P) __builtin_nontemporal_store(s_q[g * (kPix + 1) + px], &out[(((size_t)r * 8 + g) * p.D + d) * P + gp]);
      }
    } else {
#pragma unroll
      for (int a = 0; a < NPASS; ++a) {
        const int px = a * PPP + pix_in_pass;
#pragma unroll
        for (int k = 0; k < 4; ++k) {
          float avg = acc_s[a][k] / cnt;
          float avg_sq = acc_q[a][k] / cnt;
          s_out[cg * 4 + k][px] = v3d::sub_rn(avg_sq, v3d::mul_rn(avg, avg));
        }
      }
      __syncthreads();
      {
        const int px = tid % kPix;
        const int gp = ptile * kPix + px;
// ... 466 lines not shown
              const char* a = wb + (so_pl + cgb);
              t00 = *reinterpret_cast<const f32x4*>(a);
              t01 = *reinterpret_cast<const f32x4*>(a + CB);
              t10 = *reinterpret_cast<const f32x4*>(a + kWinCols * CB);
              t11 = *reinterpret_cast<const f32x4*>(a + kWinCols * CB + CB);
            }
          }
          V3D_PSV_BLEND(pl, w);
        }
      }
      skip = skip_next;
    }

    psv_wave_sync<WPB>();
    int tid_o = (int)threadIdx.x;
    if constexpr (WALK) asm volatile("" : "+v"(tid_o));
    int ne_o = ne;
    if constexpr (WALK) asm volatile("" : "+s"(ne_o));
    const float cnt = (float)max(ne_o, 1);
    const float cnt_inv = 1.f / cnt;
    if constexpr (SPLIT) {
      const int chunk = cg >> 1, half = cg & 1;
      u32x4* const out = reinterpret_cast<u32x4*>(p.var);
      const int gp = ptile * kRPix + (tid_o >> 3);
      u32x4* const obase = WALK ? out + ((size_t)r * 8 * p.D + (size_t)dchunk * kRDB) * P +
                                      ((unsigned)(chunk * 2 + half) * (unsigned)(p.D * P) + (unsigned)gp)
                                : out + (((size_t)r * 8 + chunk * 2 + half) * p.D + (size_t)dchunk * kRDB) * P + gp;
#define V3D_PSV_EMIT(MEAN)                                                                                              \
    _Pragma("unroll") for (int pl = 0; pl < kRDB; ++pl) {                                                               \
      float v[4];                                                                                                       \
      _Pragma("unroll") for (int k = 0; k < 4; ++k) {                                                                   \
        const float avg = MEAN(acc_s[pl][k]);                                                                           \
        const float avg_sq = MEAN(acc_q[pl][k]);                                                                        \
        v[k] = v3d::sub_rn(avg_sq, v3d::mul_rn(avg, avg));                                           \
      }                                                                                                                 \
      const int d = dchunk * kRDB + pl;                                                                                 \
      if constexpr (CL8) {                                                                                              \
               \
        const u32x4 slot = {__float_as_uint(v[0]), __float_as_uint(v[1]), __float_as_uint(v[2]), __float_as_uint(v[3])};\
        if (gp < P && d < p.D)                                                                                          \
          __builtin_nontemporal_store(slot, obase + (size_t)pl * (unsigned)P);                                           \
      } else {                                                                                                          \
      const unsigned h01 = pack_bf16x2(v[0], v[1]), h23 = pack_bf16x2(v[2], v[3]);                                      \
      const unsigned l01 = pack_bf16x2(v[0] - __uint_as_float(h01 << 16), v[1] - __uint_as_float(h01 & 0xffff0000u));   \
      const unsigned l23 = pack_bf16x2(v[2] - __uint_as_float(h23 << 16), v[3] - __uint_as_float(h23 & 0xffff0000u));   \
      const unsigned s0 = half ? h01 : l01, s1 = half ? h23 : l23;                     \
      const unsigned r0 = (unsigned)__builtin_amdgcn_mov_dpp((int)s0, 0xB1, 0xf, 0xf, true);    \
      const unsigned r1 = (unsigned)__builtin_amdgcn_mov_dpp((int)s1, 0xB1, 0xf, 0xf, true);                            \
      const u32x4 slot = half ? (u32x4){r0, r1, l01, l23} : (u32x4){h01, h23, r0, r1};                                  \
      if (gp < P && d < p.D && (V3D_PSVW_ABLATE != 5 || slot[0] == 0x12345u))                                           \
        __builtin_nontemporal_store(slot, obase + (size_t)pl * (unsigned)P);                                             \
      }                                                                                                                 \
    }
#define V3D_MEAN_MUL(x) ((x) * cnt_inv)
#define V3D_MEAN_DIV(x) __builtin_amdgcn_div_fixupf(v3d::div_uniform((x), cnt, cnt_inv), cnt, (x))
      if (cnt_pow2) { V3D_PSV_EMIT(V3D_MEAN_MUL) } else { V3D_PSV_EMIT(V3D_MEAN_DIV) }
#undef V3D_PSV_EMIT
#undef V3D_MEAN_MUL
#undef V3D_MEAN_DIV
    } else {
      constexpr int NPX = WPB * kRPix;
      float (*const s_out)[C][NPX + 1] = reinterpret_cast<float (*)[C][NPX + 1]>(&s_win_[0][0]);
      auto mean = [&](float x) __attribute__((always_inline)) {
        return cnt_pow2 ? x * cnt_inv : __builtin_amdgcn_div_fixupf(v3d::div_uniform(x, cnt, cnt_inv), cnt, x);
      };
      const int gp0 = (ptile - wv) * kRPix;
#pragma unroll
      for (int round = 0; round < kRDB / kOutPl; ++round) {
        __syncthreads();
#pragma unroll
        for (int q = 0; q < kOutPl; ++q) {
          const int pl = round * kOutPl + q;
#pragma unroll
          for (int k = 0; k < 4; ++k) {
            const float avg = mean(acc_s[pl][k]);
            const float avg_sq = mean(acc_q[pl][k]);
            s_out[q][cg * 4 + k][wv * kRPix + gpx] = v3d::sub_rn(avg_sq, v3d::mul_rn(avg, avg));
          }
        }
        __syncthreads();
        for (int i = tid_o; i < kOutPl * C * NPX; i += 64 * WPB) {
          const int q = i / (C * NPX), c = (i / NPX) % C, px = i % NPX;
          const int gp = gp0 + px, d = dchunk * kRDB + round * kOutPl + q;
          if (gp < P && d < p.D) __builtin_nontemporal_store(s_out[q][c][px], &p.var[(((size_t)r * C + c) * p.D + d) * P + gp]);
        }
      }
      if (WALK && dchunk + 1 < c_end) __syncthreads();
    }
  }
#undef V3D_PSV_BLEND
}

__global__ __launch_bounds__(256) void psv_positions_kernel(PsvParams p, float* __restrict__ pos, float* __restrict__ world) {
  const int P = p.h * p.w;
  const long long n_vox = (long long)p.D * P;
  const long long i = (long long)blockIdx.x * 256 + threadIdx.x;
  const int r = blockIdx.y;
  if (i >= n_vox) return;
  const int d = (int)(i / P), gp = (int)(i % P), gy = gp / p.w, gx = gp % p.w;
  const float xf = (p.w > 1 && gx == p.w - 1) ? (float)(p.W - 1) : (float)((double)gx * p.x_step);
  const float yf = (p.h > 1 && gy == p.h - 1) ? (float)(p.H - 1) : (float)((double)gy * p.y_step);
  const float z = (d == p.D - 1 && p.D > 1) ? (float)p.z_end : (float)(p.z_start + (double)d * p.z_step);
  float X, Y, Z;
  v3d::world_point(p.camp + p.ref_img[r] * kCamStride, xf, yf, z, X, Y, Z);
  if (world) {
    world[((size_t)r * 3 + 0) * n_vox + i] = X;
    world[((size_t)r * 3 + 1) * n_vox + i] = Y;
    world[((size_t)r * 3 + 2) * n_vox + i] = Z;
  }
  const float Wm1 = (float)(p.W - 1), Hm1 = (float)(p.H - 1);
  const float rWm1 = (float)(1.0 / (double)(p.W - 1)), rHm1 = (float)(1.0 / (double)(p.H - 1));
  const float Wfm1 = (float)(p.Wf - 1), Hfm1 = (float)(p.Hf - 1);
  for (int e = p.edge_ofs[r]; e < p.edge_ofs[r + 1]; ++e) {
    float ix, iy;
    v3d::sample_position(p.camp + p.edge_src[e] * kCamStride + 24, X, Y, Z, Wm1, rWm1, Hm1, rHm1, Wfm1, Hfm1, ix, iy);
    pos[((size_t)e * n_vox + i) * 2] = ix;
    pos[((size_t)e * n_vox + i) * 2 + 1] = iy;
  }
}

}

int v3d::transpose_channel_last(const float* feat, float* featT, int n_img, int C, int HW, hipStream_t s) {
  dim3 tg((HW + kPix - 1) / kPix, n_img);
  v3d::TimedScope ts("transpose_channel_last", s);
  if (C == 32) transpose_channel_last_kernel<32><<<tg, 256, 0, s>>>(feat, featT, HW);
  else if (C == 16) transpose_channel_last_kernel<16><<<tg, 256, 0, s>>>(feat, featT, HW);
  else return -1;
  return 0;
}

static size_t psv_feat_bytes(int n_img, int C, int Hf, int Wf) {
  return ((size_t)n_img * (Hf + 2) * (Wf + 2) + kTailCells(Wf)) * C * sizeof(float);
}

extern "C" size_t v3d_psv_workspace_bytes(int n_img, int C, int Hf, int Wf) {
  return v3d::align_up(psv_feat_bytes(n_img, C, Hf, Wf), 256) + v3d::align_up((size_t)n_img * kCamStride * sizeof(float), 256);
}

static int psv_walk_chunks(int forced, int n_dchunk, int n_ref, int n_ptile) {
  constexpr long long kResident = 256 * 4 * V3D_PSV_WAVES, kMinRounds = 16;
  long long walk = forced > 0 ? forced : (long long)n_ref * n_dchunk * n_ptile / (kMinRounds * kResident);
  walk = walk < 1 ? 1 : walk > n_dchunk ? n_dchunk : walk;
  if (forced > 0) return (int)walk;
  const long long n_dseg = (n_dchunk + walk - 1) / walk;
  return (int)((n_dchunk + n_dseg - 1) / n_dseg);
}

extern "C" int v3d_psv_walk_chunks(int n_ref, int D, int h, int w) {
  V3D_REQUIRE(n_ref > 0 && D > 0 && h > 0 && w > 0, V3D_ERR_BAD_SHAPE, "v3d_psv_walk_chunks: bad shape");
  return psv_walk_chunks(v3d::option(v3d::kOptPsvWalk), (D + kRDB - 1) / kRDB, n_ref, (h * w + kRPix - 1) / kRPix);
}

static int psv_variance_impl(int mode, const float* feat, const float* K, const float* R,
                                    const float* t, const int32_t* ref_img,
                                    const int32_t* edge_ofs, const int32_t* edge_src, int n_img,
                                    int n_ref, int n_edges, int C, int Hf, int Wf, int H, int W,
                                    double depth_start, double depth_interval, int D, int h, int w,
                                    float* var, void* workspace, size_t workspace_bytes,
                                    void* stream) {
  const bool split = mode != 0, cl8 = mode == 2;
  V3D_REQUIRE(feat && K && R && t && ref_img && edge_ofs && edge_src && var && workspace,
              V3D_ERR_BAD_ARG, "v3d_psv_variance_f32: null pointer argument");
  V3D_REQUIRE(C == 32 || C == 16, V3D_ERR_UNSUPPORTED,
              "v3d_psv_variance_f32: C=%d unsupported (16 or 32)", C);
  V3D_REQUIRE(W <= (1 << 20) && H <= (1 << 20), V3D_ERR_BAD_SHAPE, "v3d_psv_variance_f32: image size out of range");
  V3D_REQUIRE(!split || C == 32, V3D_ERR_UNSUPPORTED,
              "v3d_psv_variance_split: C=%d unsupported (the split layout is defined for 32 channels)", C);
  V3D_REQUIRE(n_img > 0 && n_ref > 0 && n_edges >= 0 && Hf > 0 && Wf > 0 && H > 1 && W > 1 &&
                  D > 0 && h > 0 && w > 0,
              V3D_ERR_BAD_SHAPE, "v3d_psv_variance_f32: bad shape");
  V3D_REQUIRE(Hf < 32760 && Wf < 32760, V3D_ERR_BAD_SHAPE, "v3d_psv_variance_f32: feature maps larger than 32759 cells per axis");
  V3D_REQUIRE(psv_feat_bytes(n_img, C, Hf, Wf) < (size_t)1 << 32, V3D_ERR_BAD_SHAPE,
              "v3d_psv_variance_f32: bordered feature maps exceed 4 GB (32-bit byte offsets)");
  V3D_REQUIRE(workspace_bytes >= v3d_psv_workspace_bytes(n_img, C, Hf, Wf),
              V3D_ERR_WORKSPACE_TOO_SMALL, "v3d_psv_variance_f32: workspace %zu < %zu",
              workspace_bytes, v3d_psv_workspace_bytes(n_img, C, Hf, Wf));
  hipStream_t s = (hipStream_t)stream;
  float* featT = (float*)workspace;
  float* camp = (float*)((char*)workspace + v3d::align_up(psv_feat_bytes(n_img, C, Hf, Wf), 256));
  {
    v3d::TimedScope ts("transpose_channel_last", s);
    const dim3 tg(((Hf + 2) * (Wf + 2) + kPix - 1) / kPix, n_img);
    if (C == 32) transpose_bordered_kernel<32><<<tg, 256, 0, s>>>(feat, featT, Hf, Wf, n_img);
    else transpose_bordered_kernel<16><<<tg, 256, 0, s>>>(feat, featT, Hf, Wf, n_img);
  }
  V3D_CHECK_LAUNCH("transpose_bordered_kernel");
  cam_setup_kernel<<<(n_img + 63) / 64, 64, 0, s>>>(K, R, t, camp, n_img);
  V3D_CHECK_LAUNCH("cam_setup_kernel");

  PsvParams p;
  p.featT = featT; p.K = K; p.R = R; p.t = t;
  p.ref_img = ref_img; p.edge_ofs = edge_ofs; p.edge_src = edge_src; p.var = var; p.camp = camp;
  p.n_img = n_img; p.n_ref = n_ref; p.Hf = Hf; p.Wf = Wf; p.H = H; p.W = W; p.D = D;
  p.h = h; p.w = w;
  p.n_ptile = (h * w + 15) / 16;
  p.x_step = w > 1 ? (double)(W - 1) / (double)(w - 1) : 0.0;
  p.y_step = h > 1 ? (double)(H - 1) / (double)(h - 1) : 0.0;
  const double depth_end = depth_start + (double)(D - 1) * depth_interval;
  p.z_start = depth_start;
  p.z_step = D > 1 ? (depth_end - depth_start) / (double)(D - 1) : 0.0;
  p.z_end = depth_end;
  const int n_dchunk = (D + kDB - 1) / kDB;
  const long long blocks = (long long)n_ref * n_dchunk * p.n_ptile;
  V3D_REQUIRE(blocks < (1ll << 31), V3D_ERR_BAD_SHAPE, "v3d_psv_variance_f32: grid too large");
  {
    v3d::TimedScope ts("psv_variance", s);
    const unsigned grid = (unsigned)blocks;
    const int psv_kernel = v3d::option(v3d::kOptPsvKernel);
    const bool plain_gather = psv_kernel == 2;
    if (C == 32 && !plain_gather) {
      const long long rblocks = (long long)n_ref * ((D + kRDB - 1) / kRDB) * ((h * w + kRPix - 1) / kRPix);
      V3D_REQUIRE(rblocks < (1ll << 31), V3D_ERR_BAD_SHAPE, "v3d_psv_variance_f32: grid too large");
      p.n_ptile = (h * w + kRPix - 1) / kRPix;
      const bool reuse_env = psv_kernel == 1 || kRDB != 8;
      const bool no_window = reuse_env || psv_feat_bytes(n_img, C, Hf, Wf) >= ((size_t)1 << 31);
      V3D_REQUIRE(!cl8 || !no_window, V3D_ERR_UNSUPPORTED,
                  "v3d_psv_variance_cl8: only the window kernel writes this layout (feature maps < 2 GB, no developer switch)");
      unsigned wblocks = 0;
      {
        const unsigned ndc = (unsigned)((D + kRDB - 1) / kRDB);
        const unsigned npt = (unsigned)(split || cl8 ? p.n_ptile : (p.n_ptile + 3) / 4);
        p.n_dchunk = (int)ndc;
        p.walk = psv_walk_chunks(v3d::option(v3d::kOptPsvWalk), (int)ndc, n_ref, p.n_ptile);
        if ((split || cl8) && 8ull * D * h * w >= (1ull << 32)) p.walk = 1;
        p.n_dseg = ((int)ndc + p.walk - 1) / p.walk;
        p.skip = v3d::option(v3d::kOptPsvSkip) != 0;
        const unsigned long long nblk = (unsigned long long)n_ref * p.n_dseg * npt;
        wblocks = (unsigned)nblk;
        p.rWm1 = (float)(1.0 / (double)(W - 1));
        p.rHm1 = (float)(1.0 / (double)(H - 1));
        p.m_dseg = v3d::magic_u32(nblk, (unsigned)p.n_dseg);
        p.m_ptile = v3d::magic_u32(nblk / p.n_dseg + 1, npt);
        p.m_w = v3d::magic_u32((unsigned long long)h * w + 4 * kRPix, (unsigned)w);
      }
      const bool walk = p.walk > 1;
      if (cl8) {
        if (walk) psv_variance_window_kernel<true, true, true><<<wblocks, 64, 0, s>>>(p);
        else psv_variance_window_kernel<true, true, false><<<wblocks, 64, 0, s>>>(p);
      } else if (split) {
        if (no_window) psv_variance_reuse_kernel<true><<<(unsigned)rblocks, 64, 0, s>>>(p);
        else if (walk) psv_variance_window_kernel<true, false, true><<<wblocks, 64, 0, s>>>(p);
        else psv_variance_window_kernel<true, false, false><<<wblocks, 64, 0, s>>>(p);
      } else {
        p.n_ptile = (p.n_ptile + 3) / 4;
        const long long fblocks = (long long)n_ref * ((D + kRDB - 1) / kRDB) * p.n_ptile;
        if (no_window) psv_variance_reuse_kernel<false><<<(unsigned)fblocks, 256, 0, s>>>(p);
        else if (walk) psv_variance_window_kernel<false, false, true><<<wblocks, 256, 0, s>>>(p);
        else psv_variance_window_kernel<false, false, false><<<wblocks, 256, 0, s>>>(p);
      }
    } else if (cl8) {
      return v3d::fail(V3D_ERR_UNSUPPORTED, "v3d_psv_variance_cl8: C=%d unsupported (32) / option psv_kernel = 2", C);
    } else if (split) psv_variance_kernel<32, true><<<grid, 64, 0, s>>>(p);
    else if (C == 32) psv_variance_kernel<32, false><<<grid, 64, 0, s>>>(p);
    else psv_variance_kernel<16, false><<<grid, 64, 0, s>>>(p);
  }
  V3D_CHECK_LAUNCH("psv_variance_kernel");
  return V3D_OK;
}

extern "C" int v3d_psv_sample_positions_f32(const float* K, const float* R, const float* t, const int32_t* ref_img,
                                            const int32_t* edge_ofs, const int32_t* edge_src, int n_img, int n_ref,
                                            int n_edges, int Hf, int Wf, int H, int W, double depth_start,
                                            double depth_interval, int D, int h, int w, float* pos, float* world,
                                            void* workspace, size_t workspace_bytes, void* stream) {
  V3D_REQUIRE(K && R && t && ref_img && edge_ofs && edge_src && pos && workspace, V3D_ERR_BAD_ARG,
              "v3d_psv_sample_positions_f32: null pointer argument");
  V3D_REQUIRE(n_img > 0 && n_ref > 0 && n_edges >= 0 && Hf > 0 && Wf > 0 && H > 1 && W > 1 && D > 0 && h > 0 && w > 0,
              V3D_ERR_BAD_SHAPE, "v3d_psv_sample_positions_f32: bad shape");
  V3D_REQUIRE(workspace_bytes >= (size_t)n_img * kCamStride * sizeof(float), V3D_ERR_WORKSPACE_TOO_SMALL,
              "v3d_psv_sample_positions_f32: workspace too small (n_img * 36 floats)");
  hipStream_t s = (hipStream_t)stream;
  float* camp = (float*)workspace;
  cam_setup_kernel<<<(n_img + 63) / 64, 64, 0, s>>>(K, R, t, camp, n_img);
  PsvParams p;
  memset(&p, 0, sizeof(p));
  p.ref_img = ref_img; p.edge_ofs = edge_ofs; p.edge_src = edge_src; p.camp = camp;
  p.n_img = n_img; p.n_ref = n_ref; p.Hf = Hf; p.Wf = Wf; p.H = H; p.W = W; p.D = D; p.h = h; p.w = w;
  p.x_step = w > 1 ? (double)(W - 1) / (double)(w - 1) : 0.0;
  p.y_step = h > 1 ? (double)(H - 1) / (double)(h - 1) : 0.0;
  const double depth_end = depth_start + (double)(D - 1) * depth_interval;
  p.z_start = depth_start;
  p.z_step = D > 1 ? (depth_end - depth_start) / (double)(D - 1) : 0.0;
  p.z_end = depth_end;
  const long long n_vox = (long long)D * h * w;
  psv_positions_kernel<<<dim3((unsigned)((n_vox + 255) / 256), n_ref), 256, 0, s>>>(p, pos, world);
  V3D_CHECK_LAUNCH("psv_positions_kernel");
  return V3D_OK;
}

extern "C" int v3d_psv_variance_f32(const float* feat, const float* K, const float* R, const float* t,
                                    const int32_t* ref_img, const int32_t* edge_ofs, const int32_t* edge_src,
                                    int n_img, int n_ref, int n_edges, int C, int Hf, int Wf, int H, int W,
                                    double depth_start, double depth_interval, int D, int h, int w, float* var,
                                    void* workspace, size_t workspace_bytes, void* stream) {
  return psv_variance_impl(0, feat, K, R, t, ref_img, edge_ofs, edge_src, n_img, n_ref, n_edges, C, Hf, Wf, H, W,
                           depth_start, depth_interval, D, h, w, var, workspace, workspace_bytes, stream);
}

extern "C" int v3d_psv_variance_split(const float* feat, const float* K, const float* R, const float* t,
                                      const int32_t* ref_img, const int32_t* edge_ofs, const int32_t* edge_src,
                                      int n_img, int n_ref, int n_edges, int C, int Hf, int Wf, int H, int W,
                                      double depth_start, double depth_interval, int D, int h, int w,
                                      void* var_split, void* workspace, size_t workspace_bytes, void* stream) {
  return psv_variance_impl(1, feat, K, R, t, ref_img, edge_ofs, edge_src, n_img, n_ref, n_edges, C, Hf, Wf, H, W,
                           depth_start, depth_interval, D, h, w, (float*)var_split, workspace, workspace_bytes,
                           stream);
}

extern "C" int v3d_psv_variance_cl8(const float* feat, const float* K, const float* R, const float* t,
                                    const int32_t* ref_img, const int32_t* edge_ofs, const int32_t* edge_src,
                                    int n_img, int n_ref, int n_edges, int C, int Hf, int Wf, int H, int W,
                                    double depth_start, double depth_interval, int D, int h, int w,
                                    float* var_cl8, void* workspace, size_t workspace_bytes, void* stream) {
  return psv_variance_impl(2, feat, K, R, t, ref_img, edge_ofs, edge_src, n_img, n_ref, n_edges, C, Hf, Wf, H, W,
                           depth_start, depth_interval, D, h, w, var_cl8, workspace, workspace_bytes, stream);
}

#ifdef V3D_PHASE_TIMING
extern "C" int v3d_debug_psv_phase_read(unsigned long long* out8_host, int n_blocks) {
  V3D_CHECK_HIP(hipDeviceSynchronize());
  std::vector<unsigned long long> h((size_t)8 * kPhaseSlots);
  V3D_CHECK_HIP(hipMemcpyFromSymbol(h.data(), HIP_SYMBOL(g_psv_phase), h.size() * sizeof(unsigned long long)));
  for (int i = 0; i < 8; ++i) out8_host[i] = 0;
  for (int b = 0; b < n_blocks && b < kPhaseSlots; ++b)
    for (int i = 0; i < 8; ++i) out8_host[i] += h[(size_t)b * 8 + i];
  return V3D_OK;
}
#endif
```

### 3dvnet_amd/mvsnet.py

```python
import ctypes
import os

import numpy as np
import torch
import torch.nn as nn

from . import _lib


class _Workspace:

    def __init__(self):
        self._bufs = {}
        self.tags = {}

    def get(self, name, nbytes, device):
        buf = self._bufs.get(name)
        if buf is None or buf.numel() < nbytes or buf.device != device:
            buf = torch.empty(max(int(nbytes), 256), dtype=torch.uint8, device=device)
            self._bufs[name] = buf
            self.tags.pop(name, None)
        return buf

    def __deepcopy__(self, memo):
# ... 111 lines not shown
        if self._handle is not None:
            _lib.load().v3d_costreg_free(self._handle)
            self._handle = None

    def __getstate__(self):
        st = self.__dict__.copy()
        st['_handle'], st['_packed_key'] = None, None
        return st

    def __del__(self):
        try:
            self.release()
        except Exception:
            pass

    def regularize_depth(self, x, depth_vals, return_reg=False, precision=None, return_prob=False, depth_start=None,
                         depth_interval=None):
        if return_prob and (depth_start is None or depth_interval is None):
            raise ValueError('regularize_depth(return_prob=True) needs depth_start and depth_interval')
        cl8 = isinstance(x, Cl8Variance)
        split = isinstance(x, SplitVariance) and not cl8
        precision = precision or self.precision
        if split and precision != 'split_bf16':
            raise ValueError("a SplitVariance volume is the split_bf16 operand encoding; pass the fp32 volume for 'fp32'")
        if cl8 and precision != 'fp32':
            raise ValueError("a Cl8Variance volume is the input of the exact-fp32 chain; pass precision='fp32'")
        _require_cuda(x.data if (split or cl8) else x, 'CostRegNet')
        assert not self.training, 'inference only: BatchNorm is folded with running statistics'
        lib = _lib.load()
        if split or cl8:
            (B, C, D, h, w), x = x.shape, x.data
        else:
            x = x.contiguous().float()
            B, C, D, h, w = x.shape
        assert C == self.in_channels
        handle = self.packed_handle(x.device)
        depth = torch.empty((B, h, w), dtype=torch.float32, device=x.device)
        reg = torch.empty((B, D, h, w), dtype=torch.float32, device=x.device) if return_reg else None
        nbytes = lib.v3d_costreg_workspace_bytes(handle, B, D, h, w)
        ws = self._ws.get('costreg', nbytes, x.device)
        depth_vals = depth_vals.to(device=x.device, dtype=torch.float32).contiguous()
        if return_prob:
            prob = torch.empty((B, h, w), dtype=torch.float32, device=x.device)
            rc = lib.v3d_costreg_depth_prob(handle, _lib.ptr(x), _lib.LAYOUT['cl8' if cl8 else 'split' if split else 'reference'],
                                            _lib.precision_code(precision), _lib.ptr(depth_vals), float(depth_start),
                                            float(depth_interval), B, D, h, w, _lib.ptr(depth), _lib.ptr(reg), _lib.ptr(prob),
                                            _lib.ptr(ws), ws.numel(), _lib.stream_ptr(x.device))
            _lib.check(rc, 'v3d_costreg_depth_prob')
            return (depth, reg, prob) if return_reg else (depth, prob)
        if split or cl8:
            fn = lib.v3d_costreg_depth_cl8 if cl8 else lib.v3d_costreg_depth_split
            rc = fn(handle, _lib.ptr(x), _lib.ptr(depth_vals), B, D, h, w, _lib.ptr(depth),
                    _lib.ptr(reg), _lib.ptr(ws), ws.numel(), _lib.stream_ptr(x.device))
        else:
            rc = lib.v3d_costreg_depth_f32(handle, _lib.ptr(x), _lib.ptr(depth_vals), B, D, h, w, _lib.ptr(depth),
                                           _lib.ptr(reg), _lib.precision_code(precision), _lib.ptr(ws), ws.numel(),
                                           _lib.stream_ptr(x.device))
        _lib.check(rc, 'v3d_costreg_depth_cl8' if cl8 else 'v3d_costreg_depth_split' if split else 'v3d_costreg_depth_f32')
        return (depth, reg) if return_reg else depth

    def run_layer(self, layer, x, skip=None, split=False, precision='split_bf16'):
        _require_cuda(x, 'CostRegNet')
        lib = _lib.load()
        x = x.contiguous().float()
        n, _, Di, Hi, Wi = x.shape
        mod = self._layers()[layer]
        if hasattr(mod, 'deconv'):
            co, shape = mod.deconv.out_channels, (2 * Di, 2 * Hi, 2 * Wi)
        else:
            s = mod.conv.stride[0]
            co, shape = mod.conv.out_channels, tuple((d - 1) // s + 1 for d in (Di, Hi, Wi))
        out = torch.empty((n, co) + shape, dtype=torch.float32, device=x.device)
        if skip is not None:
            skip = skip.contiguous().float()
            assert skip.shape == out.shape
        if split:
            nbytes = lib.v3d_costreg_layer_split_workspace_bytes(n, x.shape[1], Di, Hi, Wi)
            ws = self._ws.get('layer_split', nbytes, x.device)
            rc = lib.v3d_costreg_layer_split_f32(self.packed_handle(x.device), layer, _lib.ptr(x), _lib.ptr(skip), n,
                                                 Di, Hi, Wi, _lib.ptr(out), _lib.ptr(ws), ws.numel(),
                                                 _lib.stream_ptr(x.device))
            _lib.check(rc, 'v3d_costreg_layer_split_f32')
            return out
        rc = lib.v3d_costreg_layer_f32(self.packed_handle(x.device), layer, _lib.ptr(x), _lib.ptr(skip), n,
                                       Di, Hi, Wi, _lib.ptr(out), _lib.precision_code(precision),
                                       _lib.stream_ptr(x.device))
        _lib.check(rc, 'v3d_costreg_layer_f32')
        return out

    def forward(self, x):
        D = x.shape[2]
        zeros = torch.zeros(D, dtype=torch.float32, device=x.device)
        _, reg = self.regularize_depth(x, zeros, return_reg=True)
        return reg.unsqueeze(1)


class EdgeCsr(tuple):
    status_ws = None

    def check(self):
        if self.status_ws is not None:
            lib = _lib.load()
            ws = self.status_ws
            _lib.check(lib.v3d_edges_csr_status(_lib.ptr(ws), ws.numel(), _lib.stream_ptr(ws.device)), 'v3d_edges_csr')
        return self


def edges_to_csr(ref_src_edges, n_ref=None, n_img=None):
    if n_ref is not None and ref_src_edges.is_cuda:
        if n_img is None:
            raise ValueError('edges_to_csr: n_img is required with n_ref')
        lib = _lib.load()
        dev = ref_src_edges.device
        e = ref_src_edges.to(torch.int64).contiguous()
        n_edges = e.shape[1]
        ref_img = torch.empty(n_ref, dtype=torch.int32, device=dev)
        edge_ofs = torch.empty(n_ref + 1, dtype=torch.int32, device=dev)
        edge_src = torch.empty(n_edges, dtype=torch.int32, device=dev)
        ws = torch.empty(lib.v3d_edges_csr_workspace_bytes(int(n_img), int(n_ref)), dtype=torch.uint8, device=dev)
        rc = lib.v3d_edges_csr(_lib.ptr(e), n_edges, int(n_img), int(n_ref), _lib.ptr(ref_img), _lib.ptr(edge_ofs),
                               _lib.ptr(edge_src), _lib.ptr(ws), ws.numel(), _lib.stream_ptr(dev))
        _lib.check(rc, 'v3d_edges_csr')
        csr = EdgeCsr((ref_img.to(torch.int64), ref_img, edge_ofs, edge_src))
        csr.status_ws = ws
        return csr
    ref_idx, gather_idx = torch.unique(ref_src_edges[0], return_inverse=True)
    n_ref = ref_idx.shape[0]
    order = torch.sort(gather_idx, stable=True).indices
    edge_src = ref_src_edges[1][order].to(torch.int32).contiguous()
    counts = torch.bincount(gather_idx, minlength=n_ref)
    edge_ofs = torch.zeros(n_ref + 1, dtype=torch.int32, device=ref_src_edges.device)
    edge_ofs[1:] = torch.cumsum(counts, 0).to(torch.int32)
    return EdgeCsr((ref_idx, ref_idx.to(torch.int32).contiguous(), edge_ofs, edge_src))


class SplitVariance:

    def __init__(self, data, shape):
        self.data, self.shape = data, tuple(shape)

    @property
    def device(self):
        return self.data.device


class Cl8Variance(SplitVariance):
    """The variance volume as fp32 in the channel-last layout of the exact-fp32 chain's conv0 (include/v3d.h,
    v3d_psv_variance_cl8): [n_ref][4 channel groups][2 halves][D][h][w] slots of 4 floats.  The numbers of the
    reference-layout tensor, bit for bit; only `CostRegNet.regularize_depth(precision='fp32')` consumes it."""


def plane_sweep_variance(features_quarter, rotmats, tvecs, K, ref_src_edges, depth_start,
                         depth_interval, n_planes, img_size, depth_img_size, workspace=None,
                         csr=None, split=False, n_ref=None, cl8=False):
    _require_cuda(features_quarter, 'plane_sweep_variance')
    lib = _lib.load()
    feat = features_quarter.contiguous().float()
    dev = feat.device
    n_img, C, Hf, Wf = feat.shape
    if csr is None:
        csr = edges_to_csr(ref_src_edges.to(dev), n_ref=n_ref, n_img=n_img)
    _, ref_img, edge_ofs, edge_src = csr
    n_ref, n_edges = ref_img.shape[0], edge_src.shape[0]
    h, w = depth_img_size
    var = torch.empty((n_ref, C, n_planes, h, w), dtype=torch.float32, device=dev)
    nbytes = lib.v3d_psv_workspace_bytes(n_img, C, Hf, Wf)
    ws = (workspace or _Workspace()).get('psv', nbytes, dev)
    Kc, Rc, tc = (x.to(dev).contiguous().float() for x in (K, rotmats, tvecs))
    fn = lib.v3d_psv_variance_cl8 if cl8 else lib.v3d_psv_variance_split if split else lib.v3d_psv_variance_f32
    rc = fn(_lib.ptr(feat), _lib.ptr(Kc), _lib.ptr(Rc), _lib.ptr(tc), _lib.ptr(ref_img),
            _lib.ptr(edge_ofs), _lib.ptr(edge_src), n_img, n_ref, n_edges, C, Hf, Wf, int(img_size[0]),
            int(img_size[1]), float(depth_start), float(depth_interval), int(n_planes), int(h), int(w),
            _lib.ptr(var), _lib.ptr(ws), ws.numel(), _lib.stream_ptr(dev))
    _lib.check(rc, 'v3d_psv_variance_cl8' if cl8 else 'v3d_psv_variance_split' if split else 'v3d_psv_variance_f32')
    return Cl8Variance(var, var.shape) if cl8 else SplitVariance(var, var.shape) if split else var


def plane_sweep_sample_positions(rotmats, tvecs, K, ref_src_edges, depth_start, depth_interval, n_planes, img_size,
                                 feat_size, depth_img_size, device):
    lib = _lib.load()
    dev = torch.device(device)
    csr = edges_to_csr(ref_src_edges.to(dev))
    _, ref_img, edge_ofs, edge_src = csr
    n_ref, n_edges = ref_img.shape[0], edge_src.shape[0]
    h, w = depth_img_size
    n_vox = n_planes * h * w
    Kc, Rc, tc = (x.to(dev).contiguous().float() for x in (K, rotmats, tvecs))
    n_img = Kc.shape[0]
    pos = torch.empty((n_edges, n_vox, 2), dtype=torch.float32, device=dev)
    world = torch.empty((n_ref, 3, n_vox), dtype=torch.float32, device=dev)
    ws = torch.empty(n_img * 36 * 4 + 256, dtype=torch.uint8, device=dev)
    rc = lib.v3d_psv_sample_positions_f32(_lib.ptr(Kc), _lib.ptr(Rc), _lib.ptr(tc), _lib.ptr(ref_img), _lib.ptr(edge_ofs),
                                          _lib.ptr(edge_src), n_img, n_ref, n_edges, int(feat_size[0]), int(feat_size[1]),
                                          int(img_size[0]), int(img_size[1]), float(depth_start), float(depth_interval),
                                          int(n_planes), int(h), int(w), _lib.ptr(pos), _lib.ptr(world), _lib.ptr(ws),
                                          ws.numel(), _lib.stream_ptr(dev))
    _lib.check(rc, 'v3d_psv_sample_positions_f32')
    return pos, world, csr


class MVSNet(nn.Module):

    def __init__(self, feat_dim=32, img_size=(240, 320), feat_extractor=None, feat_shrinker=None,
                 precision='split_bf16'):
        super().__init__()
        self.feat_dim = feat_dim
        self.img_size = img_size
        self.feat_extractor = feat_extractor
        self.feat_shrinker = feat_shrinker
        self.native_backbone = True
        self._native_backbone = None
        self.cnn_3d = CostRegNet(feat_dim, 8, precision=precision)
        self._ws = _Workspace()
        self._depth_vals = {}
        self.last_csr = None

    def depth_values(self, depth_start, depth_interval, n_planes, device):
        key = (float(depth_start), float(depth_interval), int(n_planes), str(device))
        if key not in self._depth_vals:
            depth_end = depth_start + depth_interval * (n_planes - 1)
            self._depth_vals[key] = torch.linspace(depth_start, depth_end, n_planes).to(device)
        return self._depth_vals[key]

    def cost_volume_depth(self, features_quarter, batch, depth_start, depth_interval, n_planes,
                          depth_img_size, return_intermediates=False, csr=None, precision=None, n_ref=None,
                          return_prob=False):
        precision = precision or self.cnn_3d.precision
        split = not return_intermediates and features_quarter.shape[1] == 32 and precision == 'split_bf16'
        cl8 = (not return_intermediates and features_quarter.shape[1] == 32 and precision == 'fp32'
               and features_quarter.numel() * 4 < 2 ** 31 and _psv_kernel_option() == 0)
        if csr is None:
            csr = edges_to_csr(batch.ref_src_edges.to(features_quarter.device), n_ref=n_ref, n_img=features_quarter.shape[0])
        self.last_csr = csr
        var = plane_sweep_variance(features_quarter, batch.rotmats, batch.tvecs, batch.K,
                                   batch.ref_src_edges, depth_start, depth_interval, n_planes,
                                   self.img_size, depth_img_size, workspace=self._ws, csr=csr,
                                   split=split, n_ref=n_ref, cl8=cl8)
        vals = self.depth_values(depth_start, depth_interval, n_planes, var.device)
        grid = dict(return_prob=True, depth_start=depth_start, depth_interval=depth_interval) if return_prob else {}
        if return_intermediates:
            out = self.cnn_3d.regularize_depth(var, vals, return_reg=True, precision=precision, **grid)
            return (out[0], var) + tuple(out[1:])
        return self.cnn_3d.regularize_depth(var, vals, precision=precision, **grid)

    def check_edges(self):
        if getattr(self, 'last_csr', None) is not None:
            self.last_csr.check()
        return self

    def forward(self, batch, depth_start, depth_interval, n_planes, depth_img_size, n_ref=None, return_prob=False):
        if self.feat_extractor is not None:
            if getattr(self, '_native_backbone', None) is None or self._native_backbone.fe is not self.feat_extractor \
                    or self._native_backbone.fs is not self.feat_shrinker or self._native_backbone.precision != self.cnn_3d.precision:
                from .backbone import NativeBackbone
                self._native_backbone = NativeBackbone(self.feat_extractor, self.feat_shrinker, precision=self.cnn_3d.precision)
            nb = self._native_backbone
            if self.native_backbone and nb.is_package_pair():
                why = nb.why_not(batch.images)
                if why is not None:
                    raise _lib.V3DLibraryError('MVSNet.forward: the HIP backbone cannot take this call (%s); set '
                                               '`native_backbone = False` on the MVSNet to run the stock PyTorch modules '
                                               'explicitly' % why)
                features_half, features_quarter, features_eighth, _, _ = nb(batch.images)
            else:
                features_half, features_quarter, features_eighth, _, _ = \
                    self.feat_shrinker(*self.feat_extractor(batch.images))
        else:
            features_half = getattr(batch, 'features_half', None)
            features_quarter = batch.features_quarter
            features_eighth = getattr(batch, 'features_eighth', None)
        if return_prob:
            depth_img, prob = self.cost_volume_depth(features_quarter, batch, depth_start, depth_interval,
                                                     n_planes, depth_img_size, n_ref=n_ref, return_prob=True)
            return depth_img, features_half, features_quarter, features_eighth, prob
        depth_img = self.cost_volume_depth(features_quarter, batch, depth_start, depth_interval,
                                           n_planes, depth_img_size, n_ref=n_ref)
        return depth_img, features_half, features_quarter, features_eighth


class CostVolumeGraph:

    def __init__(self, net, features_quarter, batch, depth_start, depth_interval, n_planes, depth_img_size, n_ref,
                 precision=None, warmup=2, return_prob=False):
        _require_cuda(features_quarter, 'CostVolumeGraph')
        self.net = net
        self.features_quarter = features_quarter
        self.batch = batch
        self._args = (depth_start, depth_interval, n_planes, depth_img_size)
        self._kw = dict(precision=precision, n_ref=int(n_ref))
        self.prob = None
        if return_prob:
            self._kw['return_prob'] = True
        dev = features_quarter.device
        side = torch.cuda.Stream(device=dev)
        side.wait_stream(torch.cuda.current_stream(dev))
        with torch.cuda.stream(side), torch.no_grad():
            for _ in range(max(1, warmup)):
                net.cost_volume_depth(features_quarter, batch, *self._args, **self._kw)
        torch.cuda.current_stream(dev).wait_stream(side)
        torch.cuda.synchronize(dev)
        edges_to_csr(batch.ref_src_edges, n_ref=int(n_ref), n_img=features_quarter.shape[0]).check()
        self.graph = torch.cuda.CUDAGraph()
        with torch.cuda.graph(self.graph), torch.no_grad():
            self.depth = net.cost_volume_depth(features_quarter, batch, *self._args, **self._kw)
        if return_prob:
            self.depth, self.prob = self.depth
        self._pinned = list(net._ws._bufs.values()) + list(net.cnn_3d._ws._bufs.values()) + list(net._depth_vals.values())
        self._weights_key = net.cnn_3d._packed_key
        self._weights_handle = net.cnn_3d._handle.value if net.cnn_3d._handle is not None else None

    def stale(self):
        c = self.net.cnn_3d
        cur = c._handle.value if c._handle is not None else None
        return cur != self._weights_handle or c._packed_key != self._weights_key or \
            c._packed_key != (c._packed_key[0],) + module_state_key(c)

    def update(self, features_quarter=None, rotmats=None, tvecs=None, K=None, ref_src_edges=None):
        if features_quarter is not None:
            self.features_quarter.copy_(features_quarter)
        for name, val in (('rotmats', rotmats), ('tvecs', tvecs), ('K', K), ('ref_src_edges', ref_src_edges)):
            if val is not None:
                getattr(self.batch, name).copy_(val)
        if ref_src_edges is not None:
            edges_to_csr(self.batch.ref_src_edges, n_ref=self._kw['n_ref'], n_img=self.features_quarter.shape[0]).check()

    def replay(self):
        if self.stale():
            raise RuntimeError('CostVolumeGraph: the weights of net.cnn_3d changed after capture (the packed weight image '
                               'the graph points to was released); capture a new graph')
        self.graph.replay()
        return self.depth if self.prob is None else (self.depth, self.prob)
```

### include/v3d.h

```cpp
#ifndef V3D_H_
#define V3D_H_

#include <stddef.h>
#include <stdint.h>

#ifdef __cplusplus
extern "C" {
#endif

#define V3D_OK 0
#define V3D_ERR_BAD_SHAPE (-1)
#define V3D_ERR_BAD_ARG (-2)
#define V3D_ERR_WORKSPACE_TOO_SMALL (-3)
#define V3D_ERR_HIP (-4)
#define V3D_ERR_UNSUPPORTED (-5)

#define V3D_PRECISION_SPLIT_BF16 0
#define V3D_PRECISION_FP32 1

int v3d_set_option(const char* name, int value);
int v3d_get_option(const char* name, int* value);

int v3d_version(void);
const char* v3d_last_error(void);

int v3d_timing_enable(int on);
int v3d_timing_collect(int max_entries, char* names_host, int name_stride, float* total_ms_host,
                       int* launches_host);

size_t v3d_edges_csr_workspace_bytes(int n_img, int n_ref);
int v3d_edges_csr(const int64_t* edges, int n_edges, int n_img, int n_ref, int32_t* ref_img, int32_t* edge_ofs,
                  int32_t* edge_src, void* workspace, size_t workspace_bytes, void* stream);
int v3d_edges_csr_status(const void* workspace, size_t workspace_bytes, void* stream);

size_t v3d_psv_workspace_bytes(int n_img, int C, int Hf, int Wf);
int v3d_psv_walk_chunks(int n_ref, int D, int h, int w);
int v3d_psv_variance_f32(const float* feat, const float* K, const float* R, const float* t,
                         const int32_t* ref_img, const int32_t* edge_ofs, const int32_t* edge_src,
                         int n_img, int n_ref, int n_edges, int C, int Hf, int Wf, int H, int W,
                         double depth_start, double depth_interval, int D, int h, int w,
                         float* var, void* workspace, size_t workspace_bytes, void* stream);

int v3d_psv_sample_positions_f32(const float* K, const float* R, const float* t, const int32_t* ref_img,
                                 const int32_t* edge_ofs, const int32_t* edge_src, int n_img, int n_ref, int n_edges,
                                 int Hf, int Wf, int H, int W, double depth_start, double depth_interval, int D, int h,
                                 int w, float* pos, float* world, void* workspace, size_t workspace_bytes, void* stream);

int v3d_psv_variance_split(const float* feat, const float* K, const float* R, const float* t,
                         const int32_t* ref_img, const int32_t* edge_ofs, const int32_t* edge_src,
                         int n_img, int n_ref, int n_edges, int C, int Hf, int Wf, int H, int W,
                         double depth_start, double depth_interval, int D, int h, int w,
                         void* var_split, void* workspace, size_t workspace_bytes, void* stream);

int v3d_psv_variance_cl8(const float* feat, const float* K, const float* R, const float* t,
                         const int32_t* ref_img, const int32_t* edge_ofs, const int32_t* edge_src,
                         int n_img, int n_ref, int n_edges, int C, int Hf, int Wf, int H, int W,
                         double depth_start, double depth_interval, int D, int h, int w,
                         float* var_cl8, void* workspace, size_t workspace_bytes, void* stream);

typedef struct v3d_costreg_weights v3d_costreg_weights;

int v3d_costreg_pack(const float* const* conv_weight_host, const float* const* bn_weight_host,
                     const float* const* bn_bias_host, const float* const* bn_mean_host,
                     const float* const* bn_var_host, const float* prob_weight_host,
                     const float* prob_bias_host, int in_channels, int base_channels, float bn_eps,
                     v3d_costreg_weights** out_handle);
void v3d_costreg_free(v3d_costreg_weights* handle);

size_t v3d_costreg_workspace_bytes(const v3d_costreg_weights* handle, int n_ref, int D, int h, int w);
int v3d_costreg_depth_f32(const v3d_costreg_weights* handle, const float* var,
                          const float* depth_vals, int n_ref, int D, int h, int w, float* depth,
                          float* reg, int precision, void* workspace, size_t workspace_bytes, void* stream);
int v3d_costreg_depth_split(const v3d_costreg_weights* handle, const void* var_split,
                          const float* depth_vals, int n_ref, int D, int h, int w, float* depth,
                          float* reg, void* workspace, size_t workspace_bytes, void* stream);
int v3d_costreg_depth_cl8(const v3d_costreg_weights* handle, const void* var_cl8,
                          const float* depth_vals, int n_ref, int D, int h, int w, float* depth,
                          float* reg, void* workspace, size_t workspace_bytes, void* stream);

#define V3D_LAYOUT_REFERENCE 0
#define V3D_LAYOUT_SPLIT 1
#define V3D_LAYOUT_CL8 2
int v3d_costreg_depth_prob(const v3d_costreg_weights* handle, const void* var, int in_layout, int precision,
                           const float* depth_vals, double depth_start, double depth_interval, int n_ref, int D, int h,
                           int w, float* depth, float* reg, float* prob, void* workspace, size_t workspace_bytes,
                           void* stream);
int v3d_soft_argmin_f32(const float* x_reg, const float* depth_vals, double depth_start, double depth_interval, int n, int D,
                        int h, int w, float* depth, float* prob, void* stream);
int v3d_confidence_logits_f32(const float* x_reg, const float* depth_map, double depth_start, double depth_interval, int n,
                              int D, int h, int w, float* prob, void* stream);
int v3d_probability_map_f32(const float* cv, const float* depth_map, double depth_start, double depth_interval, int n, int D,
                            int h, int w, float* prob, void* stream);

int v3d_costreg_layer_f32(const v3d_costreg_weights* handle, int layer, const float* in,
                          const float* skip, int n, int Di, int Hi, int Wi, float* out, int precision,
                          void* stream);

size_t v3d_costreg_layer_split_workspace_bytes(int n, int cin, int Di, int Hi, int Wi);
int v3d_costreg_layer_split_f32(const v3d_costreg_weights* handle, int layer, const float* in, const float* skip,
                                int n, int Di, int Hi, int Wi, float* out, void* workspace, size_t workspace_bytes,
                                void* stream);

size_t v3d_backproject_workspace_bytes(int n_img, int C, int Hf, int Wf);
int v3d_backproject_variance_f32(const float* depth, const float* feat, const float* K, const float* R,
                                 const float* t, const int32_t* ref_img, const int32_t* edge_ofs,
                                 const int32_t* edge_src, int n_img, int n_ref, int n_edges, int C,
                                 int Hf, int Wf, int H, int W, int h, int w, double offset, int n_half,
                                 float* pts, float* var, void* workspace, size_t workspace_bytes,
                                 void* stream);

typedef struct v3d_gemm_weights v3d_gemm_weights;
int v3d_gemm_pack(const float* w_host, long long stride_seg, long long stride_co, long long stride_k,
                  int n_seg, int N, int K, const float* scale_host, const float* bias_host,
                  const float* gn_w_host, const float* gn_b_host, v3d_gemm_weights** out_handle);
void v3d_gemm_free(v3d_gemm_weights* handle);
int v3d_gemm_gather_f32(const v3d_gemm_weights* handle, int M, const float* const* seg_src_host,
                        const int32_t* const* seg_idx_host, const int* seg_ld_host, int group_len,
                        int relu_in, int use_gn, float gn_eps, const float* residual, int ld_res,
                        int relu_out, float* pool, const int32_t* pool_idx, int ld_pool, float* out,
                        int ld_out, int precision, void* stream);
int v3d_sparse_conv_f32(const v3d_gemm_weights* handle, int M, const float* src, int ld_src, const int32_t* nbr,
                        long long nbr_stride, int use_gn, float gn_eps, const float* residual, int ld_res, int relu_out,
                        float* out, int ld_out, int precision, void* stream);
int v3d_fill_f32(float* ptr, size_t n, float value, void* stream);
int v3d_pointnet_input_f32(const float* pts, const float* anchor_pts, const float* pts_feat, const int64_t* edge_anchor,
                           const int64_t* edge_pt, int n_edges, int C, float* out, void* stream);

size_t v3d_hash_bytes(int n);
int v3d_hash_build(const int32_t* coords, int n, void* table, size_t table_bytes, void* stream);
int v3d_hash_status(const void* table, int n, void* stream);
int v3d_sparse_neighbors(const void* table, int n_in, const int32_t* out_coords, int n_out, int step,
                         int32_t* nbr, void* stream);
size_t v3d_sparse_interp_workspace_bytes(int n_pts, int n_hyp);
int v3d_sparse_interp_f32(const void* table, int n_in, const float* feats, int C, int tensor_stride,
                          const float* pts, const int64_t* pts_batch, int n_pts, int n_hyp,
                          const float* min_pts, float res, float* out, int ld_out, int col0,
                          void* workspace, size_t workspace_bytes, void* stream);

size_t v3d_segment_csr_workspace_bytes(int n);
int v3d_segment_csr(const int32_t* seg_id, int n, int n_seg, int32_t* perm, int32_t* offsets, void* workspace,
                    size_t workspace_bytes, void* stream);
int v3d_segment_max_f32(const float* src, int ld, const int32_t* perm, const int32_t* offsets, int n_seg, int N, float* out,
                        int ld_out, void* stream);
size_t v3d_sort_unique_workspace_bytes(int n);
int v3d_sort_unique_u64(const uint64_t* keys_in, int n, uint64_t* keys_out, int* n_unique_host,
                        void* workspace, size_t workspace_bytes, void* stream);
int v3d_strided_keys(const int32_t* coords, int n, int tensor_stride, uint64_t* keys_out, void* stream);
int v3d_unpack_coords(const uint64_t* keys, int n, int32_t* coords_out, void* stream);
size_t v3d_voxelize_workspace_bytes(void);
int v3d_voxel_keys(const float* pts, const int64_t* pts_batch, int n, float edge_len, uint64_t* keys_out,
                   void* workspace, size_t workspace_bytes, void* stream);
int v3d_voxelize_status(const void* workspace, size_t workspace_bytes, void* stream);
int v3d_lower_bound_u64(const uint64_t* sorted_unique, int n_unique, const uint64_t* queries, int n,
                        int64_t* index_out, void* stream);
int v3d_voxel_decode(const uint64_t* unique_keys, int n_unique, float edge_len, float half_edge,
                     float* anchor_pts, int32_t* anchor_idx3d, int64_t* anchor_batch, void* workspace,
                     size_t workspace_bytes, void* stream);

int v3d_decoder_head_f32(const float* act, int n_pts, int n_hyp, int C, const float* weight,
                         const float* bias, const float* offset_vals, float* preds, float* expect,
                         void* stream);

typedef struct v3d_propagation_weights v3d_propagation_weights;
int v3d_propagation_pack(const float* const* conv_weight_host, const float* const* bn_weight_host,
                         const float* const* bn_bias_host, const float* const* bn_mean_host,
                         const float* const* bn_var_host, int in_dim, int h_dim, float bn_eps,
                         v3d_propagation_weights** out_handle);
void v3d_propagation_free(v3d_propagation_weights* handle);
int v3d_propagation_up_f32(const v3d_propagation_weights* handle, const float* features, const float* depth_lo, int B, int Cf,
                           int H, int W, int h0, int w0, const int32_t* iy, const int32_t* ix, float* out, int precision, void* stream);

size_t v3d_decoder_fused_workspace_bytes(int n_pts, int n_hyp);
int v3d_decoder_fused_f32(const v3d_gemm_weights* const* layers_host, const float* head_weight, const float* head_bias,
                          const void* const* level_table_host, const int* level_n_host,
                          const float* const* level_feats_host, const int* level_C_host, const int* level_stride_host,
                          const float* const* level_min_pts_host, const float* level_res_host, const float* pts,
                          const int64_t* pts_batch, const float* pts_feat, int c_feat, int n_pts, int n_hyp,
                          const float* offset_vals, float* preds, float* expect, float* depth_inout, void* workspace,
                          size_t workspace_bytes, void* stream);

typedef struct v3d_conv_weights v3d_conv_weights;
int v3d_conv_pack(const float* w_host, const float* bias_host, int cout, int k, v3d_conv_weights** out_handle);
void v3d_conv_free(v3d_conv_weights* handle);
int v3d_conv_nhwc_f32(const v3d_conv_weights* handle, const float* x, int n, int H, int W, int cin, int taps, int relu,
                      int res_mode, const float* res, float* out, void* stream);
int v3d_depthwise_nhwc_f32(const float* x, const float* w, const float* bias, int n, int H, int W, int C, int ksize, int stride,
                           int relu, float* out, void* stream);
int v3d_stem_f32(const float* image, const float* w, const float* bias, int n, int H, int W, float* out, void* stream);
int v3d_nhwc_to_nchw_f32(const float* in, float* out, int n, int C, int HW, void* stream);

typedef struct v3d_irb_weights v3d_irb_weights;
int v3d_irb_pack(const float* w_expand, const float* b_expand, const float* w_dw, const float* b_dw, const float* w_project,
                 const float* b_project, int cin, int mid, int cout, int ksize, int stride, int residual,
                 v3d_irb_weights** out_handle);
void v3d_irb_free(v3d_irb_weights* handle);
int v3d_irb_supported(const v3d_irb_weights* handle, int H, int W);
int v3d_stem_block_pack(const float* w_stem, const float* b_stem, const float* w_dw, const float* b_dw, const float* w_pw,
                        const float* b_pw, v3d_irb_weights** out_handle);
int v3d_stem_block_f32(const v3d_irb_weights* handle, const float* image, int n, int IH, int IW, float* out, void* stream);
size_t v3d_irb_workspace_bytes(const v3d_irb_weights* handle, int n, int H, int W);
int v3d_irb_nhwc_f32(const v3d_irb_weights* handle, const float* x, int n, int H, int W, float* out, void* workspace,
                     size_t workspace_bytes, void* stream);


typedef struct v3d_fpn_weights v3d_fpn_weights;
int v3d_fpn_pack(const float* w_lateral, const float* b_lateral, const float* w_out, const float* b_out, int cin,
                 v3d_fpn_weights** out_handle);
void v3d_fpn_free(v3d_fpn_weights* handle);
int v3d_fpn_level_f32(const v3d_fpn_weights* handle, const float* x, const float* coarse_inner, int n, int H, int W,
                      float* inner_out, float* out, void* stream);

// ... 69 lines not shown
```

Measured before the change: 20260 depth maps/s.

## Fuse edge CSR build, camera setup and feature transpose into one setup kernel

A new psv_setup_kernel builds the edge CSR table, computes camera parameters, zeroes the padding tail and transposes features to channel-last, all in one launch by giving each job its own block range. The Python path calls it whenever n_ref is known, which removes separate launches and host-side edges_to_csr work. The soft-argmin kernel also gets a 16-deep software-prefetch ring of nontemporal loads and 64-thread blocks. The cost is more code paths and a large shared-memory union per setup block.

```diff
diff --git a/3dvnet_amd/_lib.py b/3dvnet_amd/_lib.py
--- a/3dvnet_amd/_lib.py
+++ b/3dvnet_amd/_lib.py
@@ -40,6 +40,8 @@
                                [c_void_p, c_void_p, c_size_t, c_void_p]),
     'v3d_psv_variance_cl8': (c_int, [c_void_p] * 7 + [c_int] * 8 + [c_double] * 2 + [c_int] * 3 +
                              [c_void_p, c_void_p, c_size_t, c_void_p]),
+    'v3d_psv_setup_variance': (c_int, [c_int] + [c_void_p] * 5 + [c_int] * 3 + [c_void_p] * 5 + [c_size_t] + [c_int] * 5 +
+                               [c_double] * 2 + [c_int] * 3 + [c_void_p, c_void_p, c_size_t, c_void_p]),
     'v3d_costreg_depth_cl8': (c_int, [c_void_p] * 3 + [c_int] * 4 + [c_void_p, c_void_p, c_void_p,
                                                                     c_size_t, c_void_p]),
     'v3d_costreg_pack': (c_int, [c_float_pp] * 5 + [c_float_p, c_float_p, c_int, c_int, c_float,
diff --git a/3dvnet_amd/csrc/costreg.hip b/3dvnet_amd/csrc/costreg.hip
--- a/3dvnet_amd/csrc/costreg.hip
+++ b/3dvnet_amd/csrc/costreg.hip
@@ -1572,11 +1572,19 @@
   out[(ng * 2 + 1) * plane + sp] = (u32x4){la.x, la.y, lb.x, lb.y};
 }
 
-__global__ __launch_bounds__(256) void soft_argmin_kernel(const float* __restrict__ reg,
-                                                          const float* __restrict__ vals,
-                                                          float* __restrict__ depth, int n, int D,
-                                                          int HW) {
-  const size_t gid = (size_t)blockIdx.x * 256 + threadIdx.x;
+#ifndef V3D_SA_PREFETCH
+#define V3D_SA_PREFETCH 16
+#endif
+#ifndef V3D_SA_THREADS
+#define V3D_SA_THREADS 64
+#endif
+constexpr int kSaThreads = V3D_SA_THREADS, kSaPrefetch = V3D_SA_PREFETCH;
+template <int PF, int NT>
+__global__ __launch_bounds__(NT) void soft_argmin_kernel(const float* __restrict__ reg,
+                                                         const float* __restrict__ vals,
+                                                         float* __restrict__ depth, int n, int D,
+                                                         int HW) {
+  const size_t gid = (size_t)blockIdx.x * NT + threadIdx.x;
   if (gid >= (size_t)n * HW) return;
   const int b = gid / HW, pix = gid % HW;
   const float* col = reg + (size_t)b * D * HW + pix;
@@ -1592,14 +1600,30 @@
     den += ex;
   };
   int d = 0;
-  for (; d + 8 <= D; d += 8) {
-    float x[8];
-#pragma unroll
-    for (int i = 0; i < 8; ++i) x[i] = __builtin_nontemporal_load(col + (size_t)(d + i) * HW);
-#pragma unroll
-    for (int i = 0; i < 8; ++i) step(x[i], vals[d + i]);
-  }
-  for (; d < D; ++d) step(col[(size_t)d * HW], vals[d]);
+  if (D >= PF) {
+    float x[PF];
+#pragma unroll
+    for (int i = 0; i < PF; ++i) x[i] = __builtin_nontemporal_load(col + (size_t)i * HW);
+    for (; d + 2 * PF <= D; d += PF) {
+#pragma unroll
+      for (int i = 0; i < PF; ++i) {
+        step(x[i], vals[d + i]);
+        x[i] = __builtin_nontemporal_load(col + (size_t)(d + PF + i) * HW);
+      }
+    }
+#pragma unroll
+    for (int i = 0; i < PF; ++i) step(x[i], vals[d + i]);
+    d += PF;
+  }
+  if (d < D) {
+    float x[PF];
+#pragma unroll
+    for (int i = 0; i < PF; ++i)
+      if (d + i < D) x[i] = col[(size_t)(d + i) * HW];
+#pragma unroll
+    for (int i = 0; i < PF; ++i)
+      if (d + i < D) step(x[i], vals[d + i]);
+  }
   const float e = num / den;
   depth[gid] = e;
 }
@@ -2040,7 +2064,8 @@
   const size_t npix = (size_t)n * H * W;
   {
     v3d::TimedScope ts("soft_argmin", s);
-    soft_argmin_kernel<<<(unsigned)((npix + 255) / 256), 256, 0, s>>>(xreg, depth_vals, depth, n, D, H * W);
+    soft_argmin_kernel<kSaPrefetch, kSaThreads><<<(unsigned)((npix + kSaThreads - 1) / kSaThreads), kSaThreads, 0, s>>>(
+        xreg, depth_vals, depth, n, D, H * W);
   }
   V3D_CHECK_LAUNCH("soft_argmin_kernel");
   return V3D_OK;
@@ -2224,7 +2249,7 @@
                                    int D, int H, int W, float* depth, float* prob, void* stream) {
   V3D_REQUIRE(x_reg && depth_vals && depth, V3D_ERR_BAD_ARG, "v3d_soft_argmin_f32: null argument");
   V3D_REQUIRE(n > 0 && D > 0 && H > 0 && W > 0 && D < (1 << 24) && (long long)H * W < (1ll << 31) &&
-                  ((long long)n * H * W + 255) / 256 < (1ll << 31),
+                  ((long long)n * H * W + kSaThreads - 1) / kSaThreads < (1ll << 31),
               V3D_ERR_BAD_SHAPE, "v3d_soft_argmin_f32: n, D, h, w = %d, %d, %d, %d", n, D, H, W);
   const float ds = (float)depth_start, di = (float)depth_interval;
   V3D_REQUIRE(!prob || (std::isfinite(ds) && std::isfinite(di) && di != 0.f), V3D_ERR_BAD_ARG,
diff --git a/3dvnet_amd/csrc/edges.hip b/3dvnet_amd/csrc/edges.hip
--- a/3dvnet_amd/csrc/edges.hip
+++ b/3dvnet_amd/csrc/edges.hip
@@ -1,118 +1,16 @@
-#include "v3d_common.h"
+#include "edges_csr.h"
 
 namespace {
 
-constexpr int kThreads = 1024, kWaves = kThreads / 64;
-
-struct CsrMeta {
-  int magic;
-  int error;
-  int n_ref;
-  int pad;
-};
-constexpr int kMagic = 0x43535231;
-constexpr int kLdsImgs = 4096, kLdsEdges = 8192;
-
-__device__ __forceinline__ int block_inclusive_sum(int v, int* s_wave, int& total) {
-  const int lane = threadIdx.x & 63, wave = threadIdx.x >> 6;
-#pragma unroll
-  for (int o = 1; o < 64; o <<= 1) {
-    const int u = __shfl_up(v, o, 64);
-    if (lane >= o) v += u;
-  }
-  __syncthreads();
-  if (lane == 63) s_wave[wave] = v;
-  __syncthreads();
-  int base = 0, tot = 0;
-#pragma unroll
-  for (int w = 0; w < kWaves; ++w) {
-    const int x = s_wave[w];
-    if (w < wave) base += x;
-    tot += x;
-  }
-  total = tot;
-  return v + base;
-}
+using namespace v3d::csr;
 
 __global__ __launch_bounds__(kThreads) void edges_csr_kernel(const long long* __restrict__ edges, int n_edges, int n_img,
                                                               int n_ref_expected, int* __restrict__ ref_img,
                                                               int* __restrict__ edge_ofs, int* __restrict__ edge_src,
                                                               CsrMeta* __restrict__ meta, int* rank,
                                                               int* __restrict__ count) {
-  __shared__ int s_wave[kWaves];
-  __shared__ int s_err;
-  __shared__ int s_rank[kLdsImgs];
-  __shared__ int s_er[kLdsEdges];
-  const bool small = n_img <= kLdsImgs && n_edges <= kLdsEdges;
-  if (small) rank = s_rank;
-  const int tid = threadIdx.x, lane = tid & 63, wave = tid >> 6;
-  const long long* const e_ref = edges;
-  const long long* const e_src = edges + n_edges;
-  if (tid == 0) s_err = 0;
-  for (int i = tid; i < n_img; i += kThreads) rank[i] = 0;
-  __syncthreads();
-  int bad = 0;
-  for (int e = tid; e < n_edges; e += kThreads) {
-    const long long r = e_ref[e], s = e_src[e];
-    if (r < 0 || r >= n_img || s < 0 || s >= n_img) bad = 1;
-    else rank[r] = 1;
-  }
-  if (bad) s_err = 2;
-  __syncthreads();
-  const int per = (n_img + kThreads - 1) / kThreads;
-  const int lo = min(tid * per, n_img), hi = min(lo + per, n_img);
-  int sum = 0;
-  for (int i = lo; i < hi; ++i) sum += rank[i];
-  int n_ref;
-  int run = block_inclusive_sum(sum, s_wave, n_ref) - sum;
-  for (int i = lo; i < hi; ++i) {
-    const int f = rank[i];
-    rank[i] = f ? run : -1;
-    if (f && run < n_ref_expected) ref_img[run] = i;
-    run += f;
-  }
-  int err = s_err | (n_ref != n_ref_expected ? 1 : 0);
-  if (tid == 0) { meta->magic = kMagic; meta->error = err; meta->n_ref = n_ref; }
-  __syncthreads();
-  if (err) {
-    for (int r = tid; r <= n_ref_expected; r += kThreads) edge_ofs[r] = 0;
-    for (int r = tid; r < n_ref_expected; r += kThreads) ref_img[r] = 0;
-    return;
-  }
-  if (small) {
-    for (int e = tid; e < n_edges; e += kThreads) s_er[e] = rank[e_ref[e]];
-    __syncthreads();
-  }
-  auto edge_rank = [&](int e) __attribute__((always_inline)) { return small ? s_er[e] : rank[e_ref[e]]; };
-  for (int r = wave; r < n_ref; r += kWaves) {
-    int c = 0;
-    for (int e0 = 0; e0 < n_edges; e0 += 64) {
-      const int e = e0 + lane;
-      const bool hit = e < n_edges && edge_rank(e) == r;
-      c += __builtin_popcountll(__ballot(hit));
-    }
-    if (lane == 0) count[r] = c;
-  }
-  __syncthreads();
-  const int per_r = (n_ref + kThreads - 1) / kThreads;
-  const int rlo = min(tid * per_r, n_ref), rhi = min(rlo + per_r, n_ref);
-  sum = 0;
-  for (int r = rlo; r < rhi; ++r) sum += count[r];
-  int n_counted;
-  run = block_inclusive_sum(sum, s_wave, n_counted) - sum;
-  for (int r = rlo; r < rhi; ++r) { edge_ofs[r] = run; run += count[r]; }
-  if (tid == 0) edge_ofs[n_ref] = n_counted;
-  __syncthreads();
-  for (int r = wave; r < n_ref; r += kWaves) {
-    int pos = edge_ofs[r];
-    for (int e0 = 0; e0 < n_edges; e0 += 64) {
-      const int e = e0 + lane;
-      const bool hit = e < n_edges && edge_rank(e) == r;
-      const unsigned long long m = __ballot(hit);
-      if (hit) edge_src[pos + __builtin_popcountll(m & ((1ull << lane) - 1ull))] = (int)e_src[e];
-      pos += __builtin_popcountll(m);
-    }
-  }
+  __shared__ CsrLds lds;
+  edges_csr_block(lds, edges, n_edges, n_img, n_ref_expected, ref_img, nullptr, edge_ofs, edge_src, meta, rank, count);
 }
 
 }
diff --git a/3dvnet_amd/csrc/edges_csr.h b/3dvnet_amd/csrc/edges_csr.h
--- /dev/null
+++ b/3dvnet_amd/csrc/edges_csr.h
@@ -0,0 +1,133 @@
+#pragma once
+#include "v3d_common.h"
+
+namespace v3d {
+namespace csr {
+
+constexpr int kThreads = 1024, kWaves = kThreads / 64;
+
+struct CsrMeta {
+  int magic;
+  int error;
+  int n_ref;
+  int pad;
+};
+constexpr int kMagic = 0x43535231;
+constexpr int kLdsImgs = 4096, kLdsEdges = 8192;
+
+__device__ __forceinline__ int block_inclusive_sum(int v, int* s_wave, int& total) {
+  const int lane = threadIdx.x & 63, wave = threadIdx.x >> 6;
+#pragma unroll
+  for (int o = 1; o < 64; o <<= 1) {
+    const int u = __shfl_up(v, o, 64);
+    if (lane >= o) v += u;
+  }
+  __syncthreads();
+  if (lane == 63) s_wave[wave] = v;
+  __syncthreads();
+  int base = 0, tot = 0;
+#pragma unroll
+  for (int w = 0; w < kWaves; ++w) {
+    const int x = s_wave[w];
+    if (w < wave) base += x;
+    tot += x;
+  }
+  total = tot;
+  return v + base;
+}
+
+struct CsrLds {
+  int wave[kWaves];
+  int err;
+  int rank[kLdsImgs];
+  int er[kLdsEdges];
+};
+
+__device__ __forceinline__ void edges_csr_block(CsrLds& lds, const long long* __restrict__ edges, int n_edges, int n_img,
+                                                int n_ref_expected, int* __restrict__ ref_img, long long* __restrict__ ref_idx,
+                                                int* __restrict__ edge_ofs, int* __restrict__ edge_src,
+                                                CsrMeta* __restrict__ meta, int* rank, int* __restrict__ count) {
+  int* const s_wave = lds.wave;
+  int& s_err = lds.err;
+  int* const s_rank = lds.rank;
+  int* const s_er = lds.er;
+  const bool small = n_img <= kLdsImgs && n_edges <= kLdsEdges;
+  if (small) rank = s_rank;
+  const int tid = threadIdx.x, lane = tid & 63, wave = tid >> 6;
+  const long long* const e_ref = edges;
+  const long long* const e_src = edges + n_edges;
+  if (tid == 0) s_err = 0;
+  for (int i = tid; i < n_img; i += kThreads) rank[i] = 0;
+  __syncthreads();
+  int bad = 0;
+  for (int e = tid; e < n_edges; e += kThreads) {
+    const long long r = e_ref[e], s = e_src[e];
+    if (r < 0 || r >= n_img || s < 0 || s >= n_img) bad = 1;
+    else rank[r] = 1;
+  }
+  if (bad) s_err = 2;
+  __syncthreads();
+  const int per = (n_img + kThreads - 1) / kThreads;
+  const int lo = min(tid * per, n_img), hi = min(lo + per, n_img);
+  int sum = 0;
+  for (int i = lo; i < hi; ++i) sum += rank[i];
+  int n_ref;
+  int run = block_inclusive_sum(sum, s_wave, n_ref) - sum;
+  for (int i = lo; i < hi; ++i) {
+    const int f = rank[i];
+    rank[i] = f ? run : -1;
+    if (f && run < n_ref_expected) {
+      ref_img[run] = i;
+      if (ref_idx) ref_idx[run] = i;
+    }
+    run += f;
+  }
+  int err = s_err | (n_ref != n_ref_expected ? 1 : 0);
+  if (tid == 0) { meta->magic = kMagic; meta->error = err; meta->n_ref = n_ref; }
+  __syncthreads();
+  if (err) {
+    for (int r = tid; r <= n_ref_expected; r += kThreads) edge_ofs[r] = 0;
+    for (int r = tid; r < n_ref_expected; r += kThreads) {
+      ref_img[r] = 0;
+      if (ref_idx) ref_idx[r] = 0;
+    }
+    return;
+  }
+  if (small) {
+    for (int e = tid; e < n_edges; e += kThreads) s_er[e] = rank[e_ref[e]];
+    __syncthreads();
+  }
+  auto edge_rank = [&](int e) __attribute__((always_inline)) { return small ? s_er[e] : rank[e_ref[e]]; };
+  for (int r = wave; r < n_ref; r += kWaves) {
+    int c = 0;
+    for (int e0 = 0; e0 < n_edges; e0 += 64) {
+      const int e = e0 + lane;
+      const bool hit = e < n_edges && edge_rank(e) == r;
+      c += __builtin_popcountll(__ballot(hit));
+    }
+    if (lane == 0) count[r] = c;
+  }
+  __syncthreads();
+  const int per_r = (n_ref + kThreads - 1) / kThreads;
+  const int rlo = min(tid * per_r, n_ref), rhi = min(rlo + per_r, n_ref);
+  sum = 0;
+  for (int r = rlo; r < rhi; ++r) sum += count[r];
+  int n_counted;
+  run = block_inclusive_sum(sum, s_wave, n_counted) - sum;
+  for (int r = rlo; r < rhi; ++r) { edge_ofs[r] = run; run += count[r]; }
+  if (tid == 0) edge_ofs[n_ref] = n_counted;
+  __syncthreads();
+  for (int r = wave; r < n_ref; r += kWaves) {
+    int pos = edge_ofs[r];
+    for (int e0 = 0; e0 < n_edges; e0 += 64) {
+      const int e = e0 + lane;
+      const bool hit = e < n_edges && edge_rank(e) == r;
+      const unsigned long long m = __ballot(hit);
+      if (hit) edge_src[pos + __builtin_popcountll(m & ((1ull << lane) - 1ull))] = (int)e_src[e];
+      pos += __builtin_popcountll(m);
+    }
+  }
+}
+
+}
+}
diff --git a/3dvnet_amd/csrc/psv_variance.hip b/3dvnet_amd/csrc/psv_variance.hip
--- a/3dvnet_amd/csrc/psv_variance.hip
+++ b/3dvnet_amd/csrc/psv_variance.hip
@@ -4,6 +4,7 @@
 
 #include "bf16_split.h"
 #include "v3d_common.h"
+#include "edges_csr.h"
 
 namespace {
 
@@ -30,6 +31,10 @@
   int skip;
 };
 
+
+typedef float f32x4 __attribute__((ext_vector_type(4)));
+typedef unsigned int u32x2 __attribute__((ext_vector_type(2)));
+typedef unsigned int u32x4 __attribute__((ext_vector_type(4)));
 
 template <int C>
 __global__ __launch_bounds__(256) void transpose_channel_last_kernel(const float* __restrict__ in,
@@ -104,10 +109,8 @@
 
 constexpr int kCamStride = 36;
 
-__global__ void cam_setup_kernel(const float* __restrict__ K, const float* __restrict__ R,
-                                 const float* __restrict__ t, float* __restrict__ camp, int n_img) {
-  const int img = blockIdx.x * blockDim.x + threadIdx.x;
-  if (img >= n_img) return;
+__device__ __forceinline__ void cam_setup_image(const float* __restrict__ K, const float* __restrict__ R,
+                                                const float* __restrict__ t, float* __restrict__ camp, int img) {
   const float* Kp = K + img * 9;
   const float* Rp = R + img * 9;
   const float* tp = t + img * 3;
@@ -134,6 +137,69 @@
     }
 }
 
+__global__ void cam_setup_kernel(const float* __restrict__ K, const float* __restrict__ R,
+                                 const float* __restrict__ t, float* __restrict__ camp, int n_img) {
+  const int img = blockIdx.x * blockDim.x + threadIdx.x;
+  if (img < n_img) cam_setup_image(K, R, t, camp, img);
+}
+
+constexpr int kSetupCells = 256;
+struct SetupParams {
+  const float* feat; float* featT;
+  const float* K; const float* R; const float* t; float* camp;
+  const long long* edges; int* ref_img; long long* ref_idx; int* edge_ofs; int* edge_src;
+  v3d::csr::CsrMeta* meta; int* rank; int* count;
+  int n_edges, n_img, n_ref, Hf, Wf, tiles_per_img;
+};
+
+template <int C>
+__global__ __launch_bounds__(v3d::csr::kThreads) void psv_setup_kernel(SetupParams p) {
+  constexpr int NT = v3d::csr::kThreads;
+  constexpr int kRow = kSetupCells + 2;
+  static_assert(kRow % 16 == 2 && NT % kSetupCells == 0 && C % (4 * (NT / kSetupCells)) == 0, "tile geometry");
+  union Lds {
+    v3d::csr::CsrLds csr;
+    float tile[C][kRow];
+  };
+  __shared__ Lds lds;
+  const int tid = threadIdx.x;
+  if (blockIdx.x == 0) {
+    v3d::csr::edges_csr_block(lds.csr, p.edges, p.n_edges, p.n_img, p.n_ref, p.ref_img, p.ref_idx, p.edge_ofs, p.edge_src, p.meta,
+                              p.rank, p.count);
+    return;
+  }
+  const int Wp = p.Wf + 2, HW = p.Hf * p.Wf, n_cell = (p.Hf + 2) * Wp;
+  if (blockIdx.x == 1) {
+    for (int img = tid; img < p.n_img; img += NT) cam_setup_image(p.K, p.R, p.t, p.camp, img);
+    float* tail = p.featT + (size_t)p.n_img * n_cell * C;
+    for (int i = tid; i < kTailCells(p.Wf) * C; i += NT) tail[i] = 0.f;
+    return;
+  }
+  const int tb = blockIdx.x - 2;
+  const int img = tb / p.tiles_per_img, q0 = (tb - img * p.tiles_per_img) * kSetupCells;
+  const float* src = p.feat + (size_t)img * C * HW;
+  float* dst = p.featT + ((size_t)img * n_cell + q0) * C;
+  {
+    const int px = tid % kSetupCells, q = q0 + px;
+    const int yb = q / Wp, xb = q - yb * Wp;
+    const bool inside = q < n_cell && yb >= 1 && yb <= p.Hf && xb >= 1 && xb <= p.Wf;
+    constexpr int kLanes = NT / kSetupCells, kPer = C / kLanes;
+    const float* sp = src + (size_t)(tid / kSetupCells) * HW + (inside ? (yb - 1) * p.Wf + xb - 1 : 0);
+    float v[kPer];
+#pragma unroll
+    for (int k = 0; k < kPer; ++k) v[k] = inside ? sp[(size_t)(k * kLanes) * HW] : 0.f;
+#pragma unroll
+    for (int k = 0; k < kPer; ++k) lds.tile[tid / kSetupCells + k * kLanes][px] = v[k];
+  }
+  __syncthreads();
+  const int n_quad = min(kSetupCells, n_cell - q0) * (C / 4);
+  for (int i = tid; i < n_quad; i += NT) {
+    const int px = i / (C / 4), c = (i % (C / 4)) * 4;
+    const f32x4 v = {lds.tile[c][px], lds.tile[c + 1][px], lds.tile[c + 2][px], lds.tile[c + 3][px]};
+    reinterpret_cast<f32x4*>(dst)[i] = v;
+  }
+}
+
 struct TapInfo {
   float w00, w01, w10, w11;
   unsigned b00;
@@ -154,9 +220,6 @@
   return ti;
 }
 
-typedef float f32x4 __attribute__((ext_vector_type(4)));
-typedef unsigned int u32x2 __attribute__((ext_vector_type(2)));
-typedef unsigned int u32x4 __attribute__((ext_vector_type(4)));
 
 using v3d::bf16_rne;
 using v3d::pack_bf16x2;
@@ -929,7 +992,14 @@
   return psv_walk_chunks(v3d::option(v3d::kOptPsvWalk), (D + kRDB - 1) / kRDB, n_ref, (h * w + kRPix - 1) / kRPix);
 }
 
-static int psv_variance_impl(int mode, const float* feat, const float* K, const float* R,
+struct SetupEdges {
+  const int64_t* edges;
+  int64_t* ref_idx;
+  int32_t *ref_img, *edge_ofs, *edge_src;
+  void* workspace;
+};
+
+static int psv_variance_impl(int mode, const SetupEdges* fused, const float* feat, const float* K, const float* R,
                                     const float* t, const int32_t* ref_img,
                                     const int32_t* edge_ofs, const int32_t* edge_src, int n_img,
                                     int n_ref, int n_edges, int C, int Hf, int Wf, int H, int W,
@@ -956,15 +1026,32 @@
   hipStream_t s = (hipStream_t)stream;
   float* featT = (float*)workspace;
   float* camp = (float*)((char*)workspace + v3d::align_up(psv_feat_bytes(n_img, C, Hf, Wf), 256));
-  {
+  if (fused) {
+    SetupParams q;
+    q.feat = feat; q.featT = featT; q.K = K; q.R = R; q.t = t; q.camp = camp;
+    q.edges = (const long long*)fused->edges; q.ref_img = fused->ref_img; q.ref_idx = (long long*)fused->ref_idx;
+    q.edge_ofs = fused->edge_ofs; q.edge_src = fused->edge_src;
+    q.meta = (v3d::csr::CsrMeta*)fused->workspace;
+    q.rank = (int*)(q.meta + 1); q.count = q.rank + n_img;
+    q.n_edges = n_edges; q.n_img = n_img; q.n_ref = n_ref; q.Hf = Hf; q.Wf = Wf;
+    q.tiles_per_img = ((Hf + 2) * (Wf + 2) + kSetupCells - 1) / kSetupCells;
+    const long long sblocks = 2 + (long long)n_img * q.tiles_per_img;
+    V3D_REQUIRE(sblocks < (1ll << 31), V3D_ERR_BAD_SHAPE, "v3d_psv_setup_variance: grid too large");
     v3d::TimedScope ts("transpose_channel_last", s);
-    const dim3 tg(((Hf + 2) * (Wf + 2) + kPix - 1) / kPix, n_img);
-    if (C == 32) transpose_bordered_kernel<32><<<tg, 256, 0, s>>>(feat, featT, Hf, Wf, n_img);
-    else transpose_bordered_kernel<16><<<tg, 256, 0, s>>>(feat, featT, Hf, Wf, n_img);
-  }
-  V3D_CHECK_LAUNCH("transpose_bordered_kernel");
-  cam_setup_kernel<<<(n_img + 63) / 64, 64, 0, s>>>(K, R, t, camp, n_img);
-  V3D_CHECK_LAUNCH("cam_setup_kernel");
+    if (C == 32) psv_setup_kernel<32><<<(unsigned)sblocks, v3d::csr::kThreads, 0, s>>>(q);
+    else psv_setup_kernel<16><<<(unsigned)sblocks, v3d::csr::kThreads, 0, s>>>(q);
+    V3D_CHECK_LAUNCH("psv_setup_kernel");
+  } else {
+    {
+      v3d::TimedScope ts("transpose_channel_last", s);
+      const dim3 tg(((Hf + 2) * (Wf + 2) + kPix - 1) / kPix, n_img);
+      if (C == 32) transpose_bordered_kernel<32><<<tg, 256, 0, s>>>(feat, featT, Hf, Wf, n_img);
+      else transpose_bordered_kernel<16><<<tg, 256, 0, s>>>(feat, featT, Hf, Wf, n_img);
+    }
+    V3D_CHECK_LAUNCH("transpose_bordered_kernel");
+    cam_setup_kernel<<<(n_img + 63) / 64, 64, 0, s>>>(K, R, t, camp, n_img);
+    V3D_CHECK_LAUNCH("cam_setup_kernel");
+  }
 
   PsvParams p;
   p.featT = featT; p.K = K; p.R = R; p.t = t;
@@ -1071,7 +1158,7 @@
                                     int n_img, int n_ref, int n_edges, int C, int Hf, int Wf, int H, int W,
                                     double depth_start, double depth_interval, int D, int h, int w, float* var,
                                     void* workspace, size_t workspace_bytes, void* stream) {
-  return psv_variance_impl(0, feat, K, R, t, ref_img, edge_ofs, edge_src, n_img, n_ref, n_edges, C, Hf, Wf, H, W,
+  return psv_variance_impl(0, nullptr, feat, K, R, t, ref_img, edge_ofs, edge_src, n_img, n_ref, n_edges, C, Hf, Wf, H, W,
                            depth_start, depth_interval, D, h, w, var, workspace, workspace_bytes, stream);
 }
 
@@ -1080,7 +1167,7 @@
                                       int n_img, int n_ref, int n_edges, int C, int Hf, int Wf, int H, int W,
                                       double depth_start, double depth_interval, int D, int h, int w,
                                       void* var_split, void* workspace, size_t workspace_bytes, void* stream) {
-  return psv_variance_impl(1, feat, K, R, t, ref_img, edge_ofs, edge_src, n_img, n_ref, n_edges, C, Hf, Wf, H, W,
+  return psv_variance_impl(1, nullptr, feat, K, R, t, ref_img, edge_ofs, edge_src, n_img, n_ref, n_edges, C, Hf, Wf, H, W,
                            depth_start, depth_interval, D, h, w, (float*)var_split, workspace, workspace_bytes,
                            stream);
 }
@@ -1090,8 +1177,26 @@
                                     int n_img, int n_ref, int n_edges, int C, int Hf, int Wf, int H, int W,
                                     double depth_start, double depth_interval, int D, int h, int w,
                                     float* var_cl8, void* workspace, size_t workspace_bytes, void* stream) {
-  return psv_variance_impl(2, feat, K, R, t, ref_img, edge_ofs, edge_src, n_img, n_ref, n_edges, C, Hf, Wf, H, W,
+  return psv_variance_impl(2, nullptr, feat, K, R, t, ref_img, edge_ofs, edge_src, n_img, n_ref, n_edges, C, Hf, Wf, H, W,
                            depth_start, depth_interval, D, h, w, var_cl8, workspace, workspace_bytes, stream);
+}
+
+extern "C" int v3d_psv_setup_variance(int layout, const float* feat, const float* K, const float* R, const float* t,
+                                      const int64_t* edges, int n_edges, int n_img, int n_ref, int32_t* ref_img,
+                                      int64_t* ref_idx, int32_t* edge_ofs, int32_t* edge_src, void* csr_workspace,
+                                      size_t csr_workspace_bytes, int C, int Hf, int Wf, int H, int W, double depth_start,
+                                      double depth_interval, int D, int h, int w, void* var, void* workspace,
+                                      size_t workspace_bytes, void* stream) {
+  V3D_REQUIRE(layout >= 0 && layout <= 2, V3D_ERR_BAD_ARG, "v3d_psv_setup_variance: layout %d (V3D_LAYOUT_*)", layout);
+  V3D_REQUIRE(edges && ref_img && edge_ofs && edge_src && csr_workspace, V3D_ERR_BAD_ARG, "v3d_psv_setup_variance: null pointer");
+  V3D_REQUIRE(n_edges > 0 && n_img > 0 && n_ref > 0 && n_ref <= n_img, V3D_ERR_BAD_SHAPE,
+              "v3d_psv_setup_variance: n_edges=%d n_img=%d n_ref=%d", n_edges, n_img, n_ref);
+  V3D_REQUIRE(csr_workspace_bytes >= v3d_edges_csr_workspace_bytes(n_img, n_ref), V3D_ERR_WORKSPACE_TOO_SMALL,
+              "v3d_psv_setup_variance: edge-table workspace %zu < %zu bytes", csr_workspace_bytes,
+              v3d_edges_csr_workspace_bytes(n_img, n_ref));
+  const SetupEdges se = {edges, ref_idx, ref_img, edge_ofs, edge_src, csr_workspace};
+  return psv_variance_impl(layout, &se, feat, K, R, t, ref_img, edge_ofs, edge_src, n_img, n_ref, n_edges, C, Hf, Wf, H, W,
+                           depth_start, depth_interval, D, h, w, (float*)var, workspace, workspace_bytes, stream);
 }
 
 #ifdef V3D_PHASE_TIMING
diff --git a/3dvnet_amd/mvsnet.py b/3dvnet_amd/mvsnet.py
--- a/3dvnet_amd/mvsnet.py
+++ b/3dvnet_amd/mvsnet.py
@@ -287,28 +287,48 @@
 
 def plane_sweep_variance(features_quarter, rotmats, tvecs, K, ref_src_edges, depth_start,
                          depth_interval, n_planes, img_size, depth_img_size, workspace=None,
-                         csr=None, split=False, n_ref=None, cl8=False):
+                         csr=None, split=False, n_ref=None, cl8=False, return_csr=False):
     _require_cuda(features_quarter, 'plane_sweep_variance')
     lib = _lib.load()
     feat = features_quarter.contiguous().float()
     dev = feat.device
     n_img, C, Hf, Wf = feat.shape
+    h, w = depth_img_size
+    nbytes = lib.v3d_psv_workspace_bytes(n_img, C, Hf, Wf)
+    ws = (workspace or _Workspace()).get('psv', nbytes, dev)
+    Kc, Rc, tc = (x.to(dev).contiguous().float() for x in (K, rotmats, tvecs))
+    if csr is None and n_ref is not None:
+        e = ref_src_edges.to(device=dev, dtype=torch.int64).contiguous()
+        n_ref, n_edges = int(n_ref), e.shape[1]
+        ref_idx = torch.empty(n_ref, dtype=torch.int64, device=dev)
+        ref_img = torch.empty(n_ref, dtype=torch.int32, device=dev)
+        edge_ofs = torch.empty(n_ref + 1, dtype=torch.int32, device=dev)
+        edge_src = torch.empty(n_edges, dtype=torch.int32, device=dev)
+        cws = torch.empty(lib.v3d_edges_csr_workspace_bytes(n_img, n_ref), dtype=torch.uint8, device=dev)
+        var = torch.empty((n_ref, C, n_planes, h, w), dtype=torch.float32, device=dev)
+        rc = lib.v3d_psv_setup_variance(
+            _lib.LAYOUT['cl8' if cl8 else 'split' if split else 'reference'], _lib.ptr(feat), _lib.ptr(Kc), _lib.ptr(Rc),
+            _lib.ptr(tc), _lib.ptr(e), n_edges, n_img, n_ref, _lib.ptr(ref_img), _lib.ptr(ref_idx), _lib.ptr(edge_ofs),
+            _lib.ptr(edge_src), _lib.ptr(cws), cws.numel(), C, Hf, Wf, int(img_size[0]), int(img_size[1]), float(depth_start),
+            float(depth_interval), int(n_planes), int(h), int(w), _lib.ptr(var), _lib.ptr(ws), ws.numel(), _lib.stream_ptr(dev))
+        _lib.check(rc, 'v3d_psv_setup_variance')
+        csr = EdgeCsr((ref_idx, ref_img, edge_ofs, edge_src))
+        csr.status_ws = cws
+        out = Cl8Variance(var, var.shape) if cl8 else SplitVariance(var, var.shape) if split else var
+        return (out, csr) if return_csr else out
     if csr is None:
         csr = edges_to_csr(ref_src_edges.to(dev), n_ref=n_ref, n_img=n_img)
     _, ref_img, edge_ofs, edge_src = csr
     n_ref, n_edges = ref_img.shape[0], edge_src.shape[0]
-    h, w = depth_img_size
     var = torch.empty((n_ref, C, n_planes, h, w), dtype=torch.float32, device=dev)
-    nbytes = lib.v3d_psv_workspace_bytes(n_img, C, Hf, Wf)
-    ws = (workspace or _Workspace()).get('psv', nbytes, dev)
-    Kc, Rc, tc = (x.to(dev).contiguous().float() for x in (K, rotmats, tvecs))
     fn = lib.v3d_psv_variance_cl8 if cl8 else lib.v3d_psv_variance_split if split else lib.v3d_psv_variance_f32
     rc = fn(_lib.ptr(feat), _lib.ptr(Kc), _lib.ptr(Rc), _lib.ptr(tc), _lib.ptr(ref_img),
             _lib.ptr(edge_ofs), _lib.ptr(edge_src), n_img, n_ref, n_edges, C, Hf, Wf, int(img_size[0]),
             int(img_size[1]), float(depth_start), float(depth_interval), int(n_planes), int(h), int(w),
             _lib.ptr(var), _lib.ptr(ws), ws.numel(), _lib.stream_ptr(dev))
     _lib.check(rc, 'v3d_psv_variance_cl8' if cl8 else 'v3d_psv_variance_split' if split else 'v3d_psv_variance_f32')
-    return Cl8Variance(var, var.shape) if cl8 else SplitVariance(var, var.shape) if split else var
+    out = Cl8Variance(var, var.shape) if cl8 else SplitVariance(var, var.shape) if split else var
+    return (out, csr) if return_csr else out
 
 
 def plane_sweep_sample_positions(rotmats, tvecs, K, ref_src_edges, depth_start, depth_interval, n_planes, img_size,
@@ -364,13 +384,13 @@
         split = not return_intermediates and features_quarter.shape[1] == 32 and precision == 'split_bf16'
         cl8 = (not return_intermediates and features_quarter.shape[1] == 32 and precision == 'fp32'
                and features_quarter.numel() * 4 < 2 ** 31 and _psv_kernel_option() == 0)
-        if csr is None:
-            csr = edges_to_csr(batch.ref_src_edges.to(features_quarter.device), n_ref=n_ref, n_img=features_quarter.shape[0])
+        if csr is None and n_ref is None:
+            csr = edges_to_csr(batch.ref_src_edges.to(features_quarter.device))
+        var, csr = plane_sweep_variance(features_quarter, batch.rotmats, batch.tvecs, batch.K,
+                                        batch.ref_src_edges, depth_start, depth_interval, n_planes,
+                                        self.img_size, depth_img_size, workspace=self._ws, csr=csr,
+                                        split=split, n_ref=n_ref, cl8=cl8, return_csr=True)
         self.last_csr = csr
-        var = plane_sweep_variance(features_quarter, batch.rotmats, batch.tvecs, batch.K,
-                                   batch.ref_src_edges, depth_start, depth_interval, n_planes,
-                                   self.img_size, depth_img_size, workspace=self._ws, csr=csr,
-                                   split=split, n_ref=n_ref, cl8=cl8)
         vals = self.depth_values(depth_start, depth_interval, n_planes, var.device)
         grid = dict(return_prob=True, depth_start=depth_start, depth_interval=depth_interval) if return_prob else {}
         if return_intermediates:
diff --git a/include/v3d.h b/include/v3d.h
--- a/include/v3d.h
+++ b/include/v3d.h
@@ -57,6 +57,12 @@
                          int n_img, int n_ref, int n_edges, int C, int Hf, int Wf, int H, int W,
                          double depth_start, double depth_interval, int D, int h, int w,
                          float* var_cl8, void* workspace, size_t workspace_bytes, void* stream);
+
+int v3d_psv_setup_variance(int layout, const float* feat, const float* K, const float* R, const float* t,
+                           const int64_t* edges, int n_edges, int n_img, int n_ref, int32_t* ref_img, int64_t* ref_idx,
+                           int32_t* edge_ofs, int32_t* edge_src, void* csr_workspace, size_t csr_workspace_bytes,
+                           int C, int Hf, int Wf, int H, int W, double depth_start, double depth_interval, int D, int h, int w,
+                           void* var, void* workspace, size_t workspace_bytes, void* stream);
 
 typedef struct v3d_costreg_weights v3d_costreg_weights;
 
```

New measurement: 20430 depth maps/s (median of 6 runs). Within noise of the previous version (+0.8%).
